# entrpn/learning-jax-sharding

Hardware: AMD Instinct MI355X
Metric: step-time ms + TFLOPS/GPU, case6 sharded attention block at 1/2/4/8 MI355X (higher is better)
Workload: dtype bf16; 1 GPU; model=case6 attention block (M=640, heads=8x64, bf16 compute, f32 params, Adam), global_batch=64, seq_len=256, parallelism=dp1, mode=train, hip_graph=True, graph_segments=1, steps_per_graph=6, warmup_steps_run=67, comm=none, grad_wire=fp32, loss=y.sum(), rules=reference

## Files before the change

learning_jax_sharding_amd/csrc/kernels/adam_common.h:

```cpp
#pragma once
#include "rowwise.h"

template <typename ST>
__device__ __forceinline__ f32x4 ld_slab4(const ST* __restrict__ p, long e) {
  if constexpr (sizeof(ST) == 4) {
    return *(const __attribute__((address_space(1))) f32x4*)(reinterpret_cast<const float*>(p) + e);
  } else {
    const u32x2 r = *(const __attribute__((address_space(1))) u32x2*)(reinterpret_cast<const bf16_t*>(p) + e);
    return unpack_bf16x4(r);
  }
}

struct AdamTensor {
  long p, g, m, v, st, sn, R, C, g_bf16, tiles_c, vec;
  long qn, sn8, qt, st8;
  long gS, g_ld, g_ss;
  long trows;
};
constexpr int kAdamMax = 32;

inline bool adam_grad_from_row(const long* r, AdamTensor& t) {
  t.g = r[1]; t.R = r[6]; t.C = r[7]; t.g_bf16 = r[8];
  t.gS = r[9]; t.g_ld = r[14]; t.g_ss = r[15];
  if (t.gS == 0) t.g_ld = t.C;
  if (t.gS > 0 && (t.g_ld < t.C || t.g_ss < 1)) return false;
  t.tiles_c = (t.C + 63) / 64;
  return true;
}
inline bool adam_grad_vec_ok(const AdamTensor& t) {
  auto al = [](long ptr, long a) { return ptr % a == 0; };
  return t.C % 4 == 0 &&
         (t.gS < 0 || (al(t.g, t.g_bf16 ? 8 : 16) && t.g_ld % 4 == 0 && (t.gS == 0 || t.g_ss % 4 == 0)));
}

template <typename ST>
__device__ __forceinline__ float slab_sum1(const ST* __restrict__ g, long gS, long ss, long i) {
  auto ld = [&](long j) {
    if constexpr (sizeof(ST) == 4) return reinterpret_cast<const float*>(g)[j];
    else return bf2f(reinterpret_cast<const bf16_t*>(g)[j]);
  };
  float acc = ld(i);
  long s = 1;
  for (; s + 3 < gS; s += 4) acc += (ld(s * ss + i) + ld((s + 1) * ss + i)) + (ld((s + 2) * ss + i) + ld((s + 3) * ss + i));
  for (; s < gS; ++s) acc += ld(s * ss + i);
  return acc;
}
template <typename ST>
__device__ __forceinline__ f32x4 slab_sum4(const ST* __restrict__ g, long gS, long ss, long i) {
  f32x4 acc = ld_slab4(g, i);
  long s = 1;
  for (; s + 3 < gS; s += 4) {
    const f32x4 v0 = ld_slab4(g, s * ss + i), v1 = ld_slab4(g, (s + 1) * ss + i);
    const f32x4 v2 = ld_slab4(g, (s + 2) * ss + i), v3 = ld_slab4(g, (s + 3) * ss + i);
    acc += (v0 + v1) + (v2 + v3);
  }
  for (; s < gS; ++s) acc += ld_slab4(g, s * ss + i);
  return acc;
}

struct StepHyper {
  float grad_scale, lr, norm, pad;
};
```

learning_jax_sharding_amd/csrc/kernels/attention.hip:

```cpp
#include "common.h"

#include <cstdlib>
#include <type_traits>

namespace {

constexpr int D = 64;
constexpr int BLK = 64;
constexpr float LOG2E = 1.4426950408889634f;
constexpr int FKR = 256;

struct FastDiv {
  unsigned m;
  int s, d;
};
static inline FastDiv make_fastdiv(int d) {
  int s = 0;
  while ((1L << s) < d) ++s;
  const unsigned long long m = ((1ULL << 32) * ((1ULL << s) - (unsigned long long)d)) / (unsigned long long)d + 1;
  return FastDiv{(unsigned)m, s, d};
}
struct AttnArgs {
  const bf16_t* q; const bf16_t* k; const bf16_t* v; const bf16_t* o; const bf16_t* dout;
  bf16_t* out;
// ... 1444 lines not shown

template <bool MASK>
__device__ __forceinline__ void fused_tile(const AttnArgs& a, const bf16_t* Qt, const bf16_t* Ot,
                                           const float* lse_s, const float* dl_s, bf16_t* dSt,
                                           const bf16x8 (&kr)[2][2], const bf16x8 (&vr)[2][2], f32x4 (&dk)[2][4],
                                           f32x4 (&dv)[2][4], int q0, int key0, int lane, const int (&offtr)[4]) {
  const int g = lane >> 4;
#pragma unroll
  for (int s2 = 0; s2 < 2; ++s2) {
    u32x4 pbu[2], sbu[2];
#pragma unroll
    for (int tt = 0; tt < 2; ++tt) {
      const int t = 2 * s2 + tt;
      const f32x4 lse = *reinterpret_cast<const f32x4*>(lse_s + 16 * t + 4 * g);
      const f32x4 ndl = *reinterpret_cast<const f32x4*>(dl_s + 16 * t + 4 * g);
      const bf16x8 q0f = frag_rows(Qt, 16 * t, 0, lane), q1f = frag_rows(Qt, 16 * t, 1, lane);
      const bf16x8 o0f = frag_rows(Ot, 16 * t, 0, lane), o1f = frag_rows(Ot, 16 * t, 1, lane);
#pragma unroll
      for (int j = 0; j < 2; ++j) {
        f32x4 s = f32x4{0.f, 0.f, 0.f, 0.f}, dp = ndl;
        s = mfma16x16x32(q0f, kr[j][0], s);
        s = mfma16x16x32(q1f, kr[j][1], s);
        dp = mfma16x16x32(o0f, vr[j][0], dp);
        dp = mfma16x16x32(o1f, vr[j][1], dp);
        float pv[4], dsv[4];
        const f32x2 sc2 = {a.scale_log2, a.scale_log2};
#pragma unroll
        for (int h = 0; h < 2; ++h) {
          const f32x2 x = pk_fms(f32x2{s[2 * h], s[2 * h + 1]}, sc2, f32x2{lse[2 * h], lse[2 * h + 1]});
          pv[2 * h] = fast_exp2(x[0]);
          pv[2 * h + 1] = fast_exp2(x[1]);
        }
        if constexpr (MASK) {
#pragma unroll
          for (int r = 0; r < 4; ++r) {
            int q = q0 + 16 * t + 4 * g + r, key = key0 + 16 * j + (lane & 15);
            bool ok = q < a.Sq && key < a.Sk && !(a.causal && key > q + a.q_offset);
            pv[r] = ok ? pv[r] : 0.f;
          }
        }
#pragma unroll
        for (int h = 0; h < 2; ++h) {
          const f32x2 d = pk_mul(f32x2{pv[2 * h], pv[2 * h + 1]}, f32x2{dp[2 * h], dp[2 * h + 1]});
          dsv[2 * h] = d[0];
          dsv[2 * h + 1] = d[1];
        }
        pbu[j][2 * tt] = pack_bf16x2(pv[0], pv[1]);
        pbu[j][2 * tt + 1] = pack_bf16x2(pv[2], pv[3]);
        sbu[j][2 * tt] = pack_bf16x2(dsv[0], dsv[1]);
        sbu[j][2 * tt + 1] = pack_bf16x2(dsv[2], dsv[3]);
        *reinterpret_cast<u32x2*>(dSt + imgS(key0 + 16 * j + (lane & 15), 4 * t + g)) =
            u32x2{sbu[j][2 * tt], sbu[j][2 * tt + 1]};
      }
    }
    bf16x8 pb[2], sb[2];
#pragma unroll
    for (int j = 0; j < 2; ++j) {
      pb[j] = __builtin_bit_cast(bf16x8, pbu[j]);
      sb[j] = __builtin_bit_cast(bf16x8, sbu[j]);
    }
#pragma unroll
    for (int dt = 0; dt < 4; ++dt) {
      bf16x8 oa = frag_tr_o(Ot, 32 * s2, offtr[dt]);
      bf16x8 qa = frag_tr_o(Qt, 32 * s2, offtr[dt]);
#pragma unroll
      for (int j = 0; j < 2; ++j) {
        dv[j][dt] = mfma16x16x32(oa, pb[j], dv[j][dt]);
        dk[j][dt] = mfma16x16x32(qa, sb[j], dk[j][dt]);
      }
    }
  }
}


__device__ __forceinline__ void fused_stamp(const AttnArgs& a, int b, int h, int wave, int lane, int k) {
#if LJS_ATTN_BWD_TRACE
  const unsigned long long t = __builtin_amdgcn_s_memtime();
  if (a.trace && lane == 0) a.trace[(((long)b * a.H + h) * (FT / 64) + wave) * 8 + k] = t;
#else
  (void)a; (void)b; (void)h; (void)wave; (void)lane; (void)k;
#endif
}

__device__ __forceinline__ void fused_delta(const bf16_t* Ot, const bf16_t* dOt, float* ndl, int tid) {
  const int row = tid >> 3, c16 = tid & 7;
  const u32x4 o = *reinterpret_cast<const u32x4*>(Ot + img16(row, c16));
  const u32x4 d = *reinterpret_cast<const u32x4*>(dOt + img16(row, c16));
  float s = dot_bf16x8(o, d);
  s += __shfl_xor(s, 1, 64);
  s += __shfl_xor(s, 2, 64);
  s += __shfl_xor(s, 4, 64);
  if (c16 == 0) ndl[row] = -s;
}

template <bool GUARD>
__device__ __forceinline__ void fused_dq(const bf16_t* Ks, const bf16_t* dSt, f32x4 (&dq)[2], int off_q,
                                         const int (&off_k)[2], int nk32) {
#pragma unroll
  for (int s2 = 0; s2 < FK / 32; ++s2) {
    if (!GUARD || s2 < nk32) {
      bf16x8 sb = frag_tr_o(dSt, 32 * s2, off_q);
#pragma unroll
      for (int i = 0; i < 2; ++i) {
        bf16x8 ka = frag_tr_o(Ks, 32 * s2, off_k[i]);
        dq[i] = mfma16x16x32(ka, sb, dq[i]);
      }
    }
  }
}

__device__ __forceinline__ void fused_dq_stage(bf16_t* img, const f32x4 (&dq)[2], float scale, int qt, int dt0,
                                               int lane) {
  const int r = 16 * qt + (lane & 15), g = lane >> 4;
#pragma unroll
  for (int i = 0; i < 2; ++i) {
    u32x2 w;
    w[0] = pack_bf16x2(dq[i][0] * scale, dq[i][1] * scale);
    w[1] = pack_bf16x2(dq[i][2] * scale, dq[i][3] * scale);
    const int c = (2 * (dt0 + i) + (g >> 1)) ^ (r & 7);
    *reinterpret_cast<u32x2*>(img + r * D + c * 8 + 4 * (g & 1)) = w;
  }
}
template <bool GUARD>
__device__ __forceinline__ void fused_dq_flush(const AttnArgs& a, const bf16_t* img, int b, int h, int q0, int tid) {
  const int r = tid >> 3, c = tid & 7;
  const u32x4 v = *reinterpret_cast<const u32x4*>(img + r * D + ((c ^ (r & 7)) << 3));
  if (!GUARD || q0 + r < a.Sq)
    *reinterpret_cast<u32x4*>(a.out3 + b * a.out3_sb + (long)(q0 + r) * a.out3_ss + h * a.out3_sh + c * 8) = v;
}

__device__ __forceinline__ void fused_dkv_out(const AttnArgs& a, bf16_t* Ks, bf16_t* Vs, const f32x4 (&dk)[2][4],
                                              const f32x4 (&dv)[2][4], int b, int h, int key0, int klim, int lane) {
#pragma unroll
  for (int j = 0; j < 2; ++j) {
    stage_rows16(Ks + key0 * D, 16 * j, dk[j], a.scale, lane);
    stage_rows16(Vs + key0 * D, 16 * j, dv[j], 1.f, lane);
  }
  flush_rows<32>(Ks + key0 * D, a.out + b * a.out_sb + h * a.out_sh, a.out_ss, key0, klim, lane);
  flush_rows<32>(Vs + key0 * D, a.out2 + b * a.out2_sb + h * a.out2_sh, a.out2_ss, key0, klim, lane);
}

template <bool KVDMA, int SW = 0>
__global__ __launch_bounds__(FT) void attn_bwd_fused_kernel(AttnArgs a) {
  __shared__ __attribute__((aligned(16))) bf16_t Ks[FK * D];
  __shared__ __attribute__((aligned(16))) bf16_t Vs[FK * D];
  __shared__ __attribute__((aligned(16))) bf16_t dSt[FK * BLK];
  __shared__ __attribute__((aligned(16))) bf16_t QO[4 * BLK * D];
  __shared__ __attribute__((aligned(16))) bf16_t Os[BLK * D];
  __shared__ __attribute__((aligned(16))) float rowc[2][2][BLK];
  __shared__ __attribute__((aligned(16))) bf16_t dQs[BLK * D];
  const int tid = threadIdx.x, lane = tid & 63, wave = tid >> 6, g = lane >> 4;
  const int h = blockIdx.x, b = blockIdx.y;
  const int key0 = wave * 32;
  auto bstamp = [&](int k) { fused_stamp(a, b, h, wave, lane, k); };
  bstamp(0);
  const bool active = key0 < a.Sk;
  const int nk32 = (a.Sk + 31) / 32;

  const bf16_t* kb = a.k + b * a.k_sb + h * a.k_sh;
  const bf16_t* vb = a.v + b * a.v_sb + h * a.v_sh;
  if constexpr (KVDMA) {
    const u32x4 rk = rsrc_u4(kb, 2 * ((long)(a.Sk - 1) * a.k_ss + D));
    const u32x4 rv = rsrc_u4(vb, 2 * ((long)(a.Sk - 1) * a.v_ss + D));
    constexpr int NWF = FT / 64;
#pragma unroll
    for (int i = 0; i < FK / 8 / NWF; ++i) {
      const int pc = wave + NWF * i;
      const int row = 8 * pc + (lane >> 3);
      const int c = ((lane & 7) ^ (((row >> 1) & 3) << 1)) * 8;
      const bool ok = row < a.Sk;
      dma_lds_x4(rk, ok ? (int)(((long)row * a.k_ss + c) * 2) : 0x7ffffff0, Ks + pc * 512);
      dma_lds_x4(rv, ok ? (int)(((long)row * a.v_ss + c) * 2) : 0x7ffffff0, Vs + pc * 512);
    }
  } else {
#pragma unroll
// ... 47 lines not shown
      vr[j][ks] = frag_rows(Vs, key0 + 16 * j, ks, lane);
    }
  const int qt = wave & 3, dt0 = 2 * (wave >> 2);
  int offtr[4];
#pragma unroll
  for (int dt = 0; dt < 4; ++dt) offtr[dt] = tr_off(16 * dt, lane);
  const int off_q = trS_off(16 * qt, lane);
  const int off_k[2] = {tr_off(16 * dt0, lane), tr_off(16 * (dt0 + 1), lane)};
  const bool wave_mask = (a.Sq % BLK) != 0 || key0 + 32 > a.Sk || a.causal;
  auto sweep = [&](auto wm, auto vs) {
    constexpr bool WM = decltype(wm)::value;
    constexpr bool VS = decltype(vs)::value;
    for (int it = 0; it < nqt; ++it) {
      const int cur = it & 1;
      const int q0 = it * BLK;
      const bool more = it + 1 < nqt;
      if (more) issue(q0 + BLK, cur ^ 1);
      const bf16_t* Qt = QO + cur * BLK * D;
      const bf16_t* Ot = QO + (2 + cur) * BLK * D;
      if (active) {
        if constexpr (WM) {
          const bool need_mask = q0 + BLK > a.Sq || key0 + 32 > a.Sk || (a.causal && key0 + 31 > q0 + a.q_offset);
          if (need_mask) fused_tile<true>(a, Qt, Ot, rowc[cur][0], rowc[cur][1], dSt, kr, vr, dk, dv, q0, key0, lane, offtr);
          else fused_tile<false>(a, Qt, Ot, rowc[cur][0], rowc[cur][1], dSt, kr, vr, dk, dv, q0, key0, lane, offtr);
        } else {
          fused_tile<false>(a, Qt, Ot, rowc[cur][0], rowc[cur][1], dSt, kr, vr, dk, dv, q0, key0, lane, offtr);
        }
      }
      asm volatile("s_waitcnt vmcnt(0)" ::: "memory");
      __syncthreads();
      if (more) finish(cur ^ 1);
      f32x4 dq[2] = {};
      if (LJS_ATTN_DQ_UNGUARD && nk32 == FK / 32) fused_dq<false>(Ks, dSt, dq, off_q, off_k, nk32);
      else fused_dq<true>(Ks, dSt, dq, off_q, off_k, nk32);
      const int qrow = q0 + 16 * qt + (lane & 15);
      if constexpr (VS) {
        fused_dq_stage(dQs, dq, a.scale, qt, dt0, lane);
      } else if (qrow < a.Sq) {
        bf16_t* rowp = a.out3 + b * a.out3_sb + (long)qrow * a.out3_ss + h * a.out3_sh;
  #pragma unroll
        for (int i = 0; i < 2; ++i) {
          u32x2 w;
          w[0] = pack_bf16x2(dq[i][0] * a.scale, dq[i][1] * a.scale);
          w[1] = pack_bf16x2(dq[i][2] * a.scale, dq[i][3] * a.scale);
          *reinterpret_cast<u32x2*>(rowp + 16 * (dt0 + i) + 4 * g) = w;
        }
      }
      __syncthreads();
      if constexpr (VS) fused_dq_flush<true>(a, dQs, b, h, q0, tid);
      if (it < 5) bstamp(2 + it);
    }
  };
  if constexpr (SW == 1) {
    (void)wave_mask;
    sweep(std::false_type{}, std::true_type{});
  } else if (a.vst == 1) {
    if (wave_mask) sweep(std::true_type{}, std::true_type{});
    else sweep(std::false_type{}, std::true_type{});
  } else {
    if (wave_mask) sweep(std::true_type{}, std::false_type{});
    else sweep(std::false_type{}, std::false_type{});
  }
  if (a.vst) {
    if (active) fused_dkv_out(a, Ks, Vs, dk, dv, b, h, key0, a.Sk, lane);
    bstamp(7);
    return;
  }
#pragma unroll
  for (int j = 0; j < 2; ++j) {
    int key = key0 + 16 * j + (lane & 15);
    if (key < a.Sk) {
      store_row_T(a.out + b * a.out_sb + (long)key * a.out_ss + h * a.out_sh, dk[j], a.scale, lane);
      store_row_T(a.out2 + b * a.out2_sb + (long)key * a.out2_ss + h * a.out2_sh, dv[j], 1.f, lane);
    }
  }
}

struct BwdProjArgs {
  const bf16_t* dy;
  const bf16_t* w;
  long dy_ld;
  int M;
  unsigned long long* steps;
};
constexpr int PJ_TS = 32;
constexpr int PJ_BK = 32;
constexpr int PJ_A = FK * PJ_BK, PJ_STAGE = PJ_A + D * PJ_BK;
constexpr int PJ_NPW = 21;
constexpr int PJ_KS = 0, PJ_VS = PJ_KS + FK * D, PJ_DST = PJ_VS + FK * D, PJ_DO = PJ_DST + FK * BLK;
constexpr int PJ_Q = PJ_DO + FK * D, PJ_OS = PJ_Q + 2 * BLK * D, PJ_ROWC = PJ_OS + BLK * D;
constexpr int PJ_LDS = PJ_ROWC + 2 * 2 * BLK * 2;
static_assert(3 * PJ_STAGE <= PJ_Q - PJ_DST, "the ring fits the dS^T and dO images");
static_assert(PJ_LDS * 2 <= 160 * 1024, "LDS");
constexpr int PJB_STAGE = D * PJ_BK;
constexpr int PJB_G = 4, PJB_AHEAD = 3, PJB_NST = (PJB_AHEAD + 1) * PJB_G;
constexpr int PJB_ROW = 2048;
static_assert((PJB_NST & (PJB_NST - 1)) == 0 && PJB_NST * PJB_STAGE <= PJ_Q - PJ_DST, "the stages fit the two images");
static_assert((PJ_LDS + PJB_ROW) * 2 <= 160 * 1024, "LDS");
template <bool BCAST>
__global__ __launch_bounds__(FT) void attn_bwd_proj_kernel(AttnArgs a, BwdProjArgs pj) {
  __shared__ __attribute__((aligned(16))) bf16_t smem[PJ_LDS + (BCAST ? PJB_ROW : 0)];
  bf16_t* const Ks = smem + PJ_KS;
  bf16_t* const Vs = smem + PJ_VS;
  bf16_t* const dSt = smem + PJ_DST;
  bf16_t* const dOi = smem + PJ_DO;
  bf16_t* const Qs = smem + PJ_Q;
  bf16_t* const Os = smem + PJ_OS;
  float* const rowc = reinterpret_cast<float*>(smem + PJ_ROWC);
  const unsigned sb = (unsigned)(uintptr_t)(LDS_PTR(const void))smem;
  const int tid = threadIdx.x, lane = tid & 63, g = lane >> 4;
  const int wave = __builtin_amdgcn_readfirstlane(tid >> 6);
  const int t = xcd_remap(blockIdx.x, gridDim.x);
  const int b = t / a.H, h = t - b * a.H;
  const int key0 = wave * 32;
  auto bstamp = [&](int k) { fused_stamp(a, b, h, wave, lane, k); };
  bstamp(0);

  const bf16_t* kb = a.k + b * a.k_sb + h * a.k_sh;
  const bf16_t* vb = a.v + b * a.v_sb + h * a.v_sh;
  const bf16_t* qb = a.q + b * a.q_sb + h * a.q_sh;
  const bf16_t* ob = a.o + b * a.o_sb + h * a.o_sh;
  const float* lse = a.lse + ((long)b * a.H + h) * FK;
  const u32x4 rk = rsrc_u4(kb, 2 * ((long)(FK - 1) * a.k_ss + D));
  const u32x4 rv = rsrc_u4(vb, 2 * ((long)(FK - 1) * a.v_ss + D));
  const u32x4 rq = rsrc_u4(qb, 2 * ((long)(FK - 1) * a.q_ss + D));
  const u32x4 ro = rsrc_u4(ob, 2 * ((long)(FK - 1) * a.o_ss + D));
  const u32x4 rl = rsrc_u4(lse, 4L * FK);
  constexpr int OOB = 0x7ffffff0;
  const int drow = 8 * wave + (lane >> 3);
  const int dchunk = ((lane & 7) ^ (((drow >> 1) & 3) << 1)) * 8;
  auto issue = [&](int q0, int buf) {
    const int r = q0 + drow;
    dma_lds_x4_at(rq, (int)(((long)r * a.q_ss + dchunk) * 2), sb + 2 * (PJ_Q + buf * BLK * D + wave * 512));
    dma_lds_x4_at(ro, (int)(((long)r * a.o_ss + dchunk) * 2), sb + 2 * (PJ_OS + wave * 512));
    if (wave == 0) dma_lds_x1_at(rl, (q0 + lane) * 4, sb + 2 * PJ_ROWC + 4 * (buf * 2 * BLK));
  };
  auto finish = [&](int buf, int blk) { fused_delta(Os, dOi + blk * BLK * D, rowc + (buf * 2 + 1) * BLK, tid); };

  {
    const int nk = pj.M / PJ_BK;
    const u32x4 ra = rsrc_u4(pj.dy + (long)b * FK * pj.dy_ld, 2 * ((long)(FK - 1) * pj.dy_ld + pj.M));
    const u32x4 rw = rsrc_u4(pj.w + (long)h * D * pj.M, 2L * D * pj.M);
    auto sstamp = [&](int k) {
#if LJS_ATTN_BWD_TRACE
      const unsigned long long ts = __builtin_amdgcn_s_memtime();
      if (pj.steps && lane == 0 && k < PJ_TS) pj.steps[(((long)b * a.H + h) * (FT / 64) + wave) * PJ_TS + k] = ts;
#else
      (void)k;
#endif
    };
    auto frag = [&](const bf16_t* img, int rb0) {
      const int row = rb0 + (lane & 15);
      return __builtin_bit_cast(bf16x8, *reinterpret_cast<const u32x4*>(
                                            img + row * PJ_BK + ((g ^ (((row >> 3) & 1) << 1)) << 3)));
    };
    f32x4 acc[BCAST ? 1 : 2][BCAST ? 1 : 4];
#pragma unroll
    for (int i = 0; i < (BCAST ? 1 : 2); ++i)
#pragma unroll
      for (int j = 0; j < (BCAST ? 1 : 4); ++j) acc[i][j] = f32x4{0.f, 0.f, 0.f, 0.f};
    const bool tw = wave < 4;
    const int pw = wave & 3;
    int va[BCAST ? 1 : 4], vw;
    if constexpr (BCAST) {
      va[0] = (pw * 512 + lane * 8) * 2;
    } else {
#pragma unroll
      for (int i = 0; i < 4; ++i) {
        const int row = 16 * (pw + 4 * i) + (lane >> 2);
        const int c = (lane & 3) ^ (((row >> 3) & 1) << 1);
        va[i] = (int)(((long)row * pj.dy_ld + 8 * c) * 2);
      }
    }
    {
      const int row = 16 * pw + (lane >> 2);
      const int c = (lane & 3) ^ (((row >> 3) & 1) << 1);
      vw = (row * pj.M + 8 * c) * 2;
    }
    const int prow = lane >> 3;
    const int pchunk = ((lane & 7) ^ (((prow >> 1) & 3) << 1)) * 8;
    auto issue_piece = [&](int j) {
      if (j < 16) {
        const int p = pw + 4 * (j >> 1);
        const int r = 8 * p + prow;
        if (j & 1) dma_lds_x4_at(rv, (int)(((long)r * a.v_ss + pchunk) * 2), sb + 2 * (PJ_VS + p * 512));
        else dma_lds_x4_at(rk, (int)(((long)r * a.k_ss + pchunk) * 2), sb + 2 * (PJ_KS + p * 512));
      } else if (j < 18) {
        const int p = pw + 4 * (j - 16);
        dma_lds_x4_at(rq, (int)(((long)(8 * p + prow) * a.q_ss + pchunk) * 2), sb + 2 * (PJ_Q + p * 512));
      } else if (j < 20) {
        const int p = pw + 4 * (j - 18);
        dma_lds_x4_at(ro, (int)(((long)(8 * p + prow) * a.o_ss + pchunk) * 2), sb + 2 * (PJ_OS + p * 512));
      } else if (pw == 0) {
        dma_lds_x1_at(rl, lane * 4, sb + 2 * PJ_ROWC);
      }
    };
    int pi = 0;
    if constexpr (BCAST) {
      const bf16_t* const rowi = smem + PJ_LDS;
      auto issue_w = [&](int kt) {
        dma_lds_x4_at(rw, kt < nk ? vw + kt * PJ_BK * 2 : OOB,
                      sb + 2 * (PJ_DST + (kt & (PJB_NST - 1)) * PJB_STAGE + pw * 512));
      };
      if (tw) {
        dma_lds_x4_at(ra, va[0], sb + 2 * (PJ_LDS + pw * 512));
#pragma unroll
        for (int kt = 0; kt < PJB_AHEAD * PJB_G; ++kt) issue_w(kt);
        static_assert(PJB_AHEAD * PJB_G == 12, "the counted wait below");
        asm volatile("s_waitcnt vmcnt(12)" ::: "memory");
      } else {
        for (; pi < PJ_NPW; ++pi) issue_piece(pi);
      }
      __builtin_amdgcn_s_barrier();
      if (tw) {
        for (int k0 = 0, gi = 0; k0 < nk; k0 += PJB_G, ++gi) {
          static_assert((PJB_AHEAD - 1) * PJB_G == 8, "the counted wait below");
          asm volatile("s_waitcnt vmcnt(8)" ::: "memory");
          asm volatile("s_waitcnt lgkmcnt(0)" ::: "memory");
          sstamp(gi);
#pragma unroll
// ... 31 lines not shown
        dma_lds_x4_at(rw, ok ? vw + ko : OOB, sb + 2 * (st + PJ_A + pw * 512));
      };
      int s0 = 0, s1 = PJ_STAGE, s2 = 2 * PJ_STAGE;
      if (tw) {
        issue_t(0, s0);
        issue_t(1, s1);
      } else {
        issue_piece(pi++);
        issue_piece(pi++);
      }
      for (int kt = 0; kt < nk; ++kt) {
        if (tw) asm volatile("s_waitcnt vmcnt(5)" ::: "memory");
        asm volatile("s_waitcnt lgkmcnt(0)" ::: "memory");
        __builtin_amdgcn_s_barrier();
        sstamp(kt);
        bf16x8 af[2], wf[4];
#pragma unroll
        for (int j = 0; j < 4; ++j) wf[j] = frag(dSt + s0 + PJ_A, 16 * j);
#pragma unroll
        for (int i = 0; i < 2; ++i) af[i] = frag(dSt + s0, 32 * wave + 16 * i);
        if (tw) issue_t(kt + 2, s2);
        else if (pi < PJ_NPW) issue_piece(pi++);
#pragma unroll
        for (int i = 0; i < 2; ++i)
#pragma unroll
          for (int j = 0; j < 4; ++j) acc[i][j] = mfma16x16x32(wf[j], af[i], acc[i][j]);
        const int sn = s0;
        s0 = s1;
        s1 = s2;
        s2 = sn;
      }
      if (!tw)
        for (; pi < PJ_NPW; ++pi) issue_piece(pi);
      asm volatile("s_waitcnt vmcnt(0)" ::: "memory");
      asm volatile("s_waitcnt lgkmcnt(0)" ::: "memory");
      __builtin_amdgcn_s_barrier();
      sstamp(nk);
#pragma unroll
      for (int i = 0; i < 2; ++i) {
        const int row = 32 * wave + 16 * i + (lane & 15);
#pragma unroll
        for (int j = 0; j < 4; ++j) {
          u32x2 w2;
          w2[0] = pack_bf16x2(acc[i][j][0], acc[i][j][1]);
          w2[1] = pack_bf16x2(acc[i][j][2], acc[i][j][3]);
          *reinterpret_cast<u32x2*>(dOi + img8(row, 4 * j + g)) = w2;
        }
      }
    }
    bstamp(6);
  }
  __syncthreads();
  finish(0, 0);
  __syncthreads();
  bstamp(1);

  f32x4 dk[2][4] = {}, dv[2][4] = {};
  bf16x8 kr[2][2], vr[2][2];
#pragma unroll
  for (int j = 0; j < 2; ++j)
#pragma unroll
    for (int ks = 0; ks < 2; ++ks) {
      kr[j][ks] = frag_rows(Ks, key0 + 16 * j, ks, lane);
      vr[j][ks] = frag_rows(Vs, key0 + 16 * j, ks, lane);
    }
  const int qt = wave & 3, dt0 = 2 * (wave >> 2);
  int offtr[4];
#pragma unroll
  for (int dt = 0; dt < 4; ++dt) offtr[dt] = tr_off(16 * dt, lane);
  const int off_q = trS_off(16 * qt, lane);
  const int off_k[2] = {tr_off(16 * dt0, lane), tr_off(16 * (dt0 + 1), lane)};
  constexpr int nqt = FK / BLK;
  for (int it = 0; it < nqt; ++it) {
    const int cur = it & 1;
    const int q0 = it * BLK;
    const bool more = it + 1 < nqt;
    if (more) issue(q0 + BLK, cur ^ 1);
    bf16_t* const dOt = dOi + it * BLK * D;
    fused_tile<false>(a, Qs + cur * BLK * D, dOt, rowc + cur * 2 * BLK, rowc + (cur * 2 + 1) * BLK, dSt, kr, vr, dk,
                      dv, q0, key0, lane, offtr);
    asm volatile("s_waitcnt vmcnt(0)" ::: "memory");
    __syncthreads();
    if (more) finish(cur ^ 1, it + 1);
    f32x4 dq[2] = {};
    fused_dq<false>(Ks, dSt, dq, off_q, off_k, FK / 32);
    fused_dq_stage(dOt, dq, a.scale, qt, dt0, lane);
    __syncthreads();
    fused_dq_flush<false>(a, dOt, b, h, q0, tid);
    bstamp(2 + it);
  }
  fused_dkv_out(a, Ks, Vs, dk, dv, b, h, key0, FK, lane);
  bstamp(7);
}

}

#define LJS_ATTN_SWITCHES(X)                                                                                  \
          \
  X(bwd_pair, 1)                                                                                              \
                                                     \
  X(dkv32, 1)                                                                                                 \
                             \
  X(dq32, 1)                                                                                                  \
                                                                             \
  X(vst, 1)                                                                                                   \
                                    \
  X(cus, 0)                                                                                                   \
                      \
  X(fwd_res, 8)                                                                                               \
                                                  \
  X(bwd_kv_dma, 2)                                                                                            \
                                                                                            \
  X(bwd_fused, 2)                                                                                             \
                                                      \
  X(bwd_proj, 2)
#define X(name, def) kSw_##name,
enum AttnSwitch { LJS_ATTN_SWITCHES(X) kSwCount };
#undef X
#define X(name, def) def,
static const int kSwDefault[kSwCount] = {LJS_ATTN_SWITCHES(X)};
static int g_sw[kSwCount] = {LJS_ATTN_SWITCHES(X)};
#undef X
LJS_API int ljs_attn_set(int which, int v) {
  if (which < 0 || which >= kSwCount) return (int)hipErrorInvalidValue;
  g_sw[which] = v < 0 ? kSwDefault[which] : v;
  return 0;
}
LJS_API int ljs_attn_get(int which) { return which < 0 || which >= kSwCount ? -1 : g_sw[which]; }
static unsigned long long* g_attn_trace = nullptr;
LJS_API void ljs_attn_set_trace(void* p) { g_attn_trace = (unsigned long long*)p; }
static unsigned long long* g_attn_trace_steps = nullptr;
LJS_API void ljs_attn_set_trace_steps(void* p) { g_attn_trace_steps = (unsigned long long*)p; }

static AttnArgs attn_args(const void* q, const void* k, const void* v, const void* o, const void* lse, const long* qs,
                          const long* ks, const long* vs, const long* os, int Sq, int Sk, int H, float scale,
                          int causal, int q_offset) {
  AttnArgs a = {};
  a.q = (const bf16_t*)q; a.k = (const bf16_t*)k; a.v = (const bf16_t*)v; a.o = (const bf16_t*)o;
  a.lse = (float*)lse;
  a.q_sb = qs[0]; a.q_ss = qs[1]; a.q_sh = qs[2];
  a.k_sb = ks[0]; a.k_ss = ks[1]; a.k_sh = ks[2];
  a.v_sb = vs[0]; a.v_ss = vs[1]; a.v_sh = vs[2];
  a.o_sb = os[0]; a.o_ss = os[1]; a.o_sh = os[2];
  a.Sq = Sq; a.Sk = Sk; a.H = H;
  a.scale = scale; a.scale_log2 = scale * LOG2E;
  a.causal = causal; a.q_offset = q_offset;
  return a;
}
static AttnArgs attn_outs(AttnArgs a, void* o1, const long* s1, void* o2 = nullptr, const long* s2 = nullptr,
                          void* o3 = nullptr, const long* s3 = nullptr) {
  a.out = (bf16_t*)o1; a.out_sb = s1[0]; a.out_ss = s1[1]; a.out_sh = s1[2];
  if (o2) { a.out2 = (bf16_t*)o2; a.out2_sb = s2[0]; a.out2_ss = s2[1]; a.out2_sh = s2[2]; }
  if (o3) { a.out3 = (bf16_t*)o3; a.out3_sb = s3[0]; a.out3_ss = s3[1]; a.out3_sh = s3[2]; }
  return a;
}
static bool none_null(std::initializer_list<const void*> ps) {
  for (const void* p : ps)
    if (!p) return false;
  return true;
}
static bool vst_ok(const void* p, long sb, long ss, long sh) {
  return (((uintptr_t)p) & 15) == 0 && sb % 8 == 0 && ss % 8 == 0 && sh % 8 == 0;
}

#define LJS_ATTN_INSTANCES(X)                    \
  X(kFwdRes8, "attn_fwd_res<8>", 512)            \
  X(kFwdRes4, "attn_fwd_res<4>", 256)            \
  X(kFwdTiled, "attn_fwd_tiled<1>", 256)         \
  X(kBwdFused00, "attn_bwd_fused<dma=0,sw=0>", FT) \
  X(kBwdFused01, "attn_bwd_fused<dma=0,sw=1>", FT) \
  X(kBwdFused10, "attn_bwd_fused<dma=1,sw=0>", FT) \
// ... 182 lines not shown
  attn_launch(p.l[0], stream, a, nullptr, p.acc_mode);
  return (int)hipGetLastError();
}

LJS_API int ljs_attn_fwd(const void* q, const void* k, const void* v, void* o, void* lse, int B, int Sq, int Sk,
                         int H, const long* qs, const long* ks, const long* vs, const long* os, float scale,
                         int causal, int q_offset, hipStream_t stream) {
  return attn_fwd_impl(q, k, v, o, lse, B, Sq, Sk, H, qs, ks, vs, os, scale, causal, q_offset, nullptr, nullptr, 0,
                       false, stream);
}

LJS_API int ljs_attn_fwd_acc(const void* q, const void* k, const void* v, void* o, void* lse, int B, int Sq, int Sk,
                             int H, const long* qs, const long* ks, const long* vs, const long* os, float scale,
                             int causal, int q_offset, void* oacc, const long* oas, int acc_mode, hipStream_t stream) {
  return attn_fwd_impl(q, k, v, o, lse, B, Sq, Sk, H, qs, ks, vs, os, scale, causal, q_offset, oacc, oas, acc_mode,
                       true, stream);
}


static int qkv_attn_fwd_impl(const void* x, long ldx, const void* w, void* qkv, void* o, void* lse, int T, int K, int N,
                             int H, float scale, void* trace, int cus, hipStream_t stream, AttnPlan* plan = nullptr) {
  QkvAttnArgs a;
  a.x = (const bf16_t*)x; a.w = (const bf16_t*)w; a.qkv = (bf16_t*)qkv; a.o = (bf16_t*)o; a.lse = (float*)lse;
  a.T = T; a.K = K; a.N = N; a.H = H; a.ldx = (int)ldx;
  a.scale_log2 = scale * LOG2E;
  a.trace = (unsigned long long*)trace;
  const AttnPlan p = qkv_attn_fwd_plan(a, ldx, cus);
  if (plan) *plan = p;
  if (plan || p.err != hipSuccess) return (int)p.err;
  ljs_launch_rec(kAttnInst[kQkvFwd].name, dim3(p.l[0].gx), p.l[0].block);
  hipLaunchKernelGGL(qkv_attn_fwd_kernel, dim3(p.l[0].gx), dim3(p.l[0].block), 0, stream, a);
  return (int)hipGetLastError();
}
LJS_API int ljs_qkv_attn_fwd(const void* x, long ldx, const void* w, void* qkv, void* o, void* lse, int T, int K, int N,
                             int H, float scale, void* trace, hipStream_t stream) {
  return qkv_attn_fwd_impl(x, ldx, w, qkv, o, lse, T, K, N, H, scale, trace, ljs_device_cus(), stream);
}

static int attn_bwd_impl(const void* q, const void* k, const void* v, const void* o, const void* dout,
                         const void* lse, void* delta, void* dq, void* dk, void* dv, int B, int Sq, int Sk, int H,
                         const long* qs, const long* ks, const long* vs, const long* os, const long* dos,
                         const long* dqs, const long* dks, const long* dvs, float scale, int causal, int q_offset,
                         hipStream_t stream, AttnPlan* plan = nullptr) {
  if (!none_null({qs, ks, vs, os, dos, dqs, dks, dvs})) return (int)hipErrorInvalidValue;
  AttnArgs a = attn_args(q, k, v, o, lse, qs, ks, vs, os, Sq, Sk, H, scale, causal, q_offset);
  a.dout = (const bf16_t*)dout;
  a.delta = (const float*)delta;
  a.do_sb = dos[0]; a.do_ss = dos[1]; a.do_sh = dos[2];
  AttnArgs f = attn_outs(a, dk, dks, dv, dvs, dq, dqs);
  const AttnPlan p = attn_bwd_plan(f, B);
  if (plan) *plan = p;
  if (plan || p.err != hipSuccess) return (int)p.err;
  if (p.l[0].inst >= kBwdFused00 && p.l[0].inst <= kBwdFused11) {
    f.vst = p.vst[0];
    f.trace = g_attn_trace;
    attn_launch(p.l[0], stream, f);
    return (int)hipGetLastError();
  }
  AttnArgs c = attn_outs(a, dq, dqs), b = attn_outs(a, dk, dks, dv, dvs);
  c.vst = p.vst[0];
  c.flags32 = p.flags32;
  b.vst = p.vst[1];
  if (p.n == 1) {
    attn_launch(p.l[0], stream, c, &b);
  } else {
    attn_launch(p.l[0], stream, c);
    attn_launch(p.l[1], stream, b);
  }
  return (int)hipGetLastError();
}
LJS_API int ljs_attn_bwd(const void* q, const void* k, const void* v, const void* o, const void* dout,
                         const void* lse, void* delta, void* dq, void* dk, void* dv, int B, int Sq, int Sk, int H,
                         const long* qs, const long* ks, const long* vs, const long* os, const long* dos,
                         const long* dqs, const long* dks, const long* dvs, float scale, int causal, int q_offset,
                         hipStream_t stream) {
  return attn_bwd_impl(q, k, v, o, dout, lse, delta, dq, dk, dv, B, Sq, Sk, H, qs, ks, vs, os, dos, dqs, dks, dvs,
                       scale, causal, q_offset, stream);
}

static int attn_bwd_proj_impl(const void* q, const void* k, const void* v, const void* o, const void* dy, long dy_ld,
                              const void* w, int M, const void* lse, void* dq, void* dk, void* dv, int B, int Sq,
                              int Sk, int H, const long* qs, const long* ks, const long* vs, const long* os,
                              const long* dqs, const long* dks, const long* dvs, float scale, int causal,
                              hipStream_t stream, AttnPlan* plan = nullptr) {
  if (!none_null({qs, ks, vs, os, dqs, dks, dvs})) return (int)hipErrorInvalidValue;
  AttnArgs a = attn_outs(attn_args(q, k, v, o, lse, qs, ks, vs, os, Sq, Sk, H, scale, causal, 0), dk, dks, dv, dvs,
                         dq, dqs);
  BwdProjArgs pj;
  pj.dy = (const bf16_t*)dy; pj.w = (const bf16_t*)w; pj.dy_ld = dy_ld; pj.M = M;
  pj.steps = g_attn_trace_steps;
  const AttnPlan p = attn_bwd_proj_plan(a, B, pj);
  if (plan) *plan = p;
  if (plan || p.err != hipSuccess) return (int)p.err;
  a.vst = p.vst[0];
  a.trace = g_attn_trace;
  ljs_launch_rec(kAttnInst[kBwdProj].name, dim3(p.l[0].gx), p.l[0].block);
  const bool bcast = dy_ld == 0 && M <= PJB_ROW && bwd_proj_bcast_on();
  g_bwd_proj_last_path = bcast;
  if (bcast) hipLaunchKernelGGL(attn_bwd_proj_kernel<true>, dim3(p.l[0].gx), dim3(p.l[0].block), 0, stream, a, pj);
  else hipLaunchKernelGGL(attn_bwd_proj_kernel<false>, dim3(p.l[0].gx), dim3(p.l[0].block), 0, stream, a, pj);
  return (int)hipGetLastError();
}
LJS_API int ljs_attn_bwd_proj_last_path() { return g_bwd_proj_last_path; }
LJS_API int ljs_attn_bwd_proj(const void* q, const void* k, const void* v, const void* o, const void* dy, long dy_ld,
                              const void* w, int M, const void* lse, void* dq, void* dk, void* dv, int B, int Sq,
                              int Sk, int H, const long* qs, const long* ks, const long* vs, const long* os,
                              const long* dqs, const long* dks, const long* dvs, float scale, int causal,
                              hipStream_t stream) {
  return attn_bwd_proj_impl(q, k, v, o, dy, dy_ld, w, M, lse, dq, dk, dv, B, Sq, Sk, H, qs, ks, vs, os, dqs, dks, dvs,
                            scale, causal, stream);
}

LJS_API int ljs_attn_plan(int kind, int B, int Sq, int Sk, int H, int causal, int acc_mode, void* const* addr,
                          const long* st, int M, long ld, int K, int cus, int* out, char* names, int cap) {
  void* const* p = addr;
  AttnPlan pl = attn_reject();
  if (kind == 0 || kind == 1)
    attn_fwd_impl(p[0], p[1], p[2], p[3], p[4], B, Sq, Sk, H, st, st + 3, st + 6, st + 9, 1.f, causal, 0, p[7],
                  kind ? st + 15 : nullptr, acc_mode, kind == 1, nullptr, &pl);
  else if (kind == 2)
    attn_bwd_impl(p[0], p[1], p[2], p[3], p[5], p[4], p[6], p[8], p[9], p[10], B, Sq, Sk, H, st, st + 3, st + 6, st + 9,
                  st + 12, st + 18, st + 21, st + 24, 1.f, causal, 0, nullptr, &pl);
  else if (kind == 3)
    attn_bwd_proj_impl(p[0], p[1], p[2], p[3], p[11], ld, p[12], M, p[4], p[8], p[9], p[10], B, Sq, Sk, H, st, st + 3,
                       st + 6, st + 9, st + 18, st + 21, st + 24, 1.f, causal, nullptr, &pl);
  else if (kind == 4)
    qkv_attn_fwd_impl(p[0], ld, p[1], p[2], p[3], p[4], B * Sq, K, M, H, 1.f, nullptr, cus, nullptr, &pl);
  const int v[16] = {(int)pl.err, pl.n, pl.l[0].inst, (int)pl.l[0].gx, (int)pl.l[0].gy, (int)pl.l[0].block,
                     pl.l[1].inst, (int)pl.l[1].gx, (int)pl.l[1].gy, (int)pl.l[1].block, pl.vst[0], pl.vst[1],
                     pl.flags32, pl.nw, pl.nqb, pl.acc_mode};
  for (int i = 0; i < 16; ++i) out[i] = v[i];
  if (names && cap > 0)
    snprintf(names, (size_t)cap, "%s%s%s", pl.n > 0 ? kAttnInst[pl.l[0].inst].name : "", pl.n > 1 ? " " : "",
             pl.n > 1 ? kAttnInst[pl.l[1].inst].name : "");
  return (int)pl.err;
}
```

learning_jax_sharding_amd/csrc/kernels/clip.hip:

```cpp
#include "adam_common.h"
#include <algorithm>
#include <math.h>

namespace {

constexpr int kSumsqRows = 32, kSumsqThreads = 256, kSumsqMaxBlocks = 1024, kSumsqSlots = 64;
constexpr int kSumsqTicketWord = kSumsqMaxBlocks;
constexpr int kSumsqSlotWord = kSumsqTicketWord + 64;
constexpr int kSumsqWsWords = kSumsqSlotWord + 2 * kSumsqSlots;
static_assert(1 + kSumsqMaxBlocks / (int)kTicketGroup <= 64 && kSumsqSlotWord % 2 == 0, "workspace layout");

struct SumsqBatch {
  AdamTensor t[kAdamMax];
  int tile_start[kAdamMax + 1];
  int n;
};

__device__ __forceinline__ void add_sq4(float& acc, const f32x4& g) {
#pragma unroll
  for (int e = 0; e < 4; ++e) acc += g[e] * g[e];
}

__global__ __launch_bounds__(kSumsqThreads) void grad_sumsq_kernel(SumsqBatch batch, float* __restrict__ partials,
                                                                    unsigned* __restrict__ tickets,
                                                                    double* __restrict__ slot) {
  const int lane = threadIdx.x & 63, w = threadIdx.x >> 6;
  const int c4 = (threadIdx.x & 15) * 4, r0 = threadIdx.x >> 4;
  const int total = batch.tile_start[batch.n];
  float acc = 0.f;
  for (int id = blockIdx.x; id < total; id += gridDim.x) {
    int ti = 0;
#pragma unroll
    for (int i = 1; i < kAdamMax; ++i) ti += (i < batch.n && id >= batch.tile_start[i]) ? 1 : 0;
    const AdamTensor& T = batch.t[ti];
    const long R = T.R, C = T.C, gS = T.gS, g_ld = T.g_ld, g_ss = T.g_ss;
    const bool bf = T.g_bf16 != 0;
    const int local = id - batch.tile_start[ti];
    const int tr_i = local / (int)T.tiles_c, tc_i = local % (int)T.tiles_c;
    if (gS >= 0 && T.vec && (long)(tc_i + 1) * 64 <= C) {
      const long cbase = (long)tc_i * 64 + c4;
      f32x4 g[2];
      bool ok[2];
#pragma unroll
      for (int q = 0; q < 2; ++q) {
        const long row = (long)tr_i * kSumsqRows + r0 + 16 * q;
        ok[q] = row < R;
        const long gi = (ok[q] ? row : 0) * g_ld + cbase;
        if (gS > 0) {
          g[q] = bf ? slab_sum4(reinterpret_cast<const bf16_t*>(T.g), gS, g_ss, gi)
                    : slab_sum4(reinterpret_cast<const float*>(T.g), gS, g_ss, gi);
        } else {
          g[q] = bf ? ld_slab4(reinterpret_cast<const bf16_t*>(T.g), gi)
                    : ld_slab4(reinterpret_cast<const float*>(T.g), gi);
        }
      }
#pragma unroll
      for (int q = 0; q < 2; ++q)
        if (ok[q]) add_sq4(acc, g[q]);
      continue;
    }
    const long col = (long)tc_i * 64 + lane;
#pragma unroll 4
    for (int rr = 0; rr < kSumsqRows / 4; ++rr) {
      const long row = (long)tr_i * kSumsqRows + w + 4 * rr;
      if (row < R && col < C) {
        const long gi = row * g_ld + col;
        const float g = gS > 0   ? (bf ? slab_sum1(reinterpret_cast<const bf16_t*>(T.g), gS, g_ss, gi)
                                       : slab_sum1(reinterpret_cast<const float*>(T.g), gS, g_ss, gi))
                        : gS < 0 ? __int_as_float((int)g_ld)
                        : bf     ? bf2f(reinterpret_cast<const bf16_t*>(T.g)[gi])
                                 : reinterpret_cast<const float*>(T.g)[gi];
        acc += g * g;
      }
    }
  }
  acc = warp_sum64(acc);
  __shared__ float part[kSumsqThreads / 64];
  if (lane == 0) part[w] = acc;
  __syncthreads();
  if (w != 0) return;
  if (lane == 0) {
    float t = part[0];
#pragma unroll
    for (int k = 1; k < kSumsqThreads / 64; ++k) t += part[k];
    sc1_store(partials + blockIdx.x, t);
  }
  if (!wave_last_2lvl(tickets, blockIdx.x, gridDim.x)) return;
  constexpr int kRounds = kSumsqMaxBlocks / 64;
  __shared__ float parked[kSumsqMaxBlocks];
  float v[kRounds];
#pragma unroll
  for (int r = 0; r < kRounds; ++r) {
    const unsigned i = r * 64 + lane;
    v[r] = i < gridDim.x ? sc1_load(partials + i) : 0.f;
  }
#pragma unroll
  for (int r = 0; r < kRounds; ++r) parked[r * 64 + lane] = v[r];
  double sum = 0.0;
#pragma unroll 1
  for (unsigned r = 0; r * 64 < gridDim.x; ++r) {
    const unsigned x = __float_as_uint(parked[r * 64 + lane]);
#pragma unroll
    for (int l = 0; l < 64; ++l) sum += (double)__uint_as_float(__builtin_amdgcn_readlane(x, l));
  }
  if (lane == 0) *slot = sum;
}

struct SchedArgs {
  int kind;
  double p[5];
};
__device__ __forceinline__ double sched_linear(double init, double end, double steps, double begin, double count) {
  if (steps <= 0.0) return init;
  const double c = fmin(fmax(count - begin, 0.0), steps);
  return (init - end) * (1.0 - c / steps) + end;
}
__device__ __forceinline__ double sched_cosine(double init, double decay_steps, double alpha, double count) {
  const double c = fmin(count, decay_steps);
  return init * ((1.0 - alpha) * 0.5 * (1.0 + cos(M_PI * c / decay_steps)) + alpha);
}
__device__ __forceinline__ double sched_value(const SchedArgs& s, double count) {
  switch (s.kind) {
    case 1: return sched_linear(s.p[0], s.p[1], s.p[2], s.p[3], count);
    case 2: return sched_cosine(s.p[0], s.p[1], s.p[2], count);
    case 3: return count < s.p[2] ? sched_linear(s.p[0], s.p[1], s.p[2], 0.0, count)
                                  : sched_cosine(s.p[1], s.p[3], s.p[4], count - s.p[2]);
    default: return s.p[0];
  }
}

__global__ __launch_bounds__(64) void step_hyper_kernel(const double* __restrict__ slots, int n_slots,
                                                        const double* __restrict__ gathered, int n_gathered,
                                                        double* __restrict__ partial_out, const int* __restrict__ step,
                                                        int step_offset, int clip, double max_norm, SchedArgs sched,
                                                        StepHyper* __restrict__ rec) {
  double s = 0.0;
  for (int i = 0; i < n_slots; ++i) s += slots[i];
  if (partial_out) {
    if (threadIdx.x == 0) *partial_out = s;
    return;
  }
  if (gathered) {
    s = 0.0;
    for (int i = 0; i < n_gathered; ++i) s += gathered[i];
  }
  const double norm = sqrt(s);
  const double scale = (!clip || norm < max_norm) ? 1.0 : max_norm / norm;
  const double count = (double)(*step + step_offset - 1);
  const double lr = sched_value(sched, count);
  if (threadIdx.x == 0) {
    rec->grad_scale = (float)scale;
// ... 51 lines not shown
```

learning_jax_sharding_amd/csrc/kernels/elementwise.hip:

```cpp
#include "adam_common.h"
#include <stdlib.h>
#include <type_traits>
#include <algorithm>

namespace {

constexpr int kMaxGrid = 2048;

inline int grid_for(long n, int per_block) {
  long g = (n + per_block - 1) / per_block;
  if (g < 1) g = 1;
  return (int)(g > kMaxGrid ? kMaxGrid : g);
}

__global__ void cast_f32_bf16(const float* __restrict__ in, bf16_t* __restrict__ out, long n) {
  long i8 = ((long)blockIdx.x * blockDim.x + threadIdx.x) * 8;
  long stride = (long)gridDim.x * blockDim.x * 8;
  for (; i8 + 8 <= n; i8 += stride) {
    float v[8];
    load_chunk8(in + i8, v);
    store_chunk(out + i8, v);
  }
  if (i8 < n) for (long j = i8; j < n; ++j) out[j] = f2bf(in[j]);
}
// ... 367 lines not shown
  int lane = threadIdx.x & 63;
  if (row >= rows) return;
  const float* x = in + row * L;
  float* y = out + row * L;
  float m = -INFINITY;
  for (int i = lane; i < L; i += 64) m = fmaxf(m, x[i]);
  m = warp_max64(m);
  float s = 0.f;
  for (int i = lane; i < L; i += 64) s += __expf(x[i] - m);
  s = warp_sum64(s);
  float inv = 1.f / s;
  for (int i = lane; i < L; i += 64) y[i] = __expf(x[i] - m) * inv;
}

template <typename G>
__global__ void adam_kernel(const float* __restrict__ p, const G* __restrict__ g, const float* __restrict__ m,
                            const float* __restrict__ v, float* __restrict__ po, float* __restrict__ mo,
                            float* __restrict__ vo, const int* __restrict__ step, long n, float lr, float b1,
                            float b2, float eps, float wd) {
  const float t = (float)(*step);
  const float bc1 = 1.f - powf(b1, t), bc2 = 1.f - powf(b2, t);
  const float inv_bc1 = 1.f / bc1, inv_sqrt_bc2 = rsqrtf(bc2);
  long i = ((long)blockIdx.x * blockDim.x + threadIdx.x) * 4;
  long stride = (long)gridDim.x * blockDim.x * 4;
  for (; i < n; i += stride) {
    if (i + 4 <= n) {
      f32x4 pp = *reinterpret_cast<const f32x4*>(p + i);
      f32x4 mm = *reinterpret_cast<const f32x4*>(m + i);
      f32x4 vv = *reinterpret_cast<const f32x4*>(v + i);
      f32x4 gg;
#pragma unroll
      for (int k = 0; k < 4; ++k) gg[k] = load1(g + i + k);
#pragma unroll
      for (int k = 0; k < 4; ++k) {
        mm[k] = b1 * mm[k] + (1.f - b1) * gg[k];
        vv[k] = b2 * vv[k] + (1.f - b2) * gg[k] * gg[k];
        float u = (mm[k] * inv_bc1) / (sqrtf(vv[k]) * inv_sqrt_bc2 + eps) + wd * pp[k];
        pp[k] -= lr * u;
      }
      *reinterpret_cast<f32x4*>(po + i) = pp;
      *reinterpret_cast<f32x4*>(mo + i) = mm;
      *reinterpret_cast<f32x4*>(vo + i) = vv;
    } else {
      for (long j = i; j < n; ++j) {
        float gg = load1(g + j);
        float mm = b1 * m[j] + (1.f - b1) * gg;
        float vv = b2 * v[j] + (1.f - b2) * gg * gg;
        float u = (mm * inv_bc1) / (sqrtf(vv) * inv_sqrt_bc2 + eps) + wd * p[j];
        po[j] = p[j] - lr * u;
        mo[j] = mm;
        vo[j] = vv;
      }
    }
  }
}

#ifndef LJS_ADAM_SLAB_DB
#define LJS_ADAM_SLAB_DB 1
#endif
struct AdamBatch {
  AdamTensor t[kAdamMax];
  int tile_start[kAdamMax + 1];
  int n;
};


struct CastJob {
  const float* src;
  bf16_t* dst;
  long n;
};

__device__ __forceinline__ float scaled_grad(float g, float scale) {
  g *= scale;
  asm volatile("" : "+v"(g));
  return g;
}

template <int kAdamRows, int kThreads, bool kDyn = false>
__global__ __launch_bounds__(kThreads) void adam_multi_kernel(AdamBatch batch, int* __restrict__ step, int step_offset,
                                                         std::conditional_t<kDyn, const StepHyper*, float> lr_arg,
                                                         float b1, float b2, float eps, float wd, CastJob cast) {
  __shared__ float tr[kAdamRows][65];
  float lr;
  [[maybe_unused]] float gscale = 1.f;
  if constexpr (kDyn) {
    gscale = lr_arg->grad_scale;
    lr = lr_arg->lr;
  } else {
    lr = lr_arg;
  }
  const int id = blockIdx.x;
  if (cast.n > 0 && id >= batch.tile_start[batch.n]) {
    const int cb = id - batch.tile_start[batch.n], ncb = (int)gridDim.x - batch.tile_start[batch.n];
    long i8 = ((long)cb * kThreads + threadIdx.x) * 8;
    const long stride = (long)ncb * kThreads * 8;
    for (; i8 + 8 <= cast.n; i8 += stride) {
      float v[8];
      load_chunk8(cast.src + i8, v);
      store_chunk(cast.dst + i8, v);
    }
    if (i8 < cast.n)
      for (long j = i8; j < cast.n; ++j) cast.dst[j] = f2bf(cast.src[j]);
    return;
  }
  int ti = 0;
#pragma unroll
  for (int i = 1; i < kAdamMax; ++i) ti += (i < batch.n && id >= batch.tile_start[i]) ? 1 : 0;
  const AdamTensor T = batch.t[ti];
  const int local = id - batch.tile_start[ti];
  const int tr_i = local / (int)T.tiles_c, tc_i = local % (int)T.tiles_c;
  const int s0 = *step;
  const float t = (float)(s0 + step_offset);
  const float inv_bc1 = 1.f / (1.f - powf(b1, t)), inv_sqrt_bc2 = rsqrtf(1.f - powf(b2, t));
  float* P = reinterpret_cast<float*>(T.p);
  float* Mm = reinterpret_cast<float*>(T.m);
  float* Vv = reinterpret_cast<float*>(T.v);
  const int tx = threadIdx.x & 63, ty = threadIdx.x >> 6;
  const int col = tc_i * 64 + tx;
  constexpr int RPP = kThreads / 16;
  auto vec_tile = [&](auto nq_tag) {
    constexpr int NQ = decltype(nq_tag)::value;
    constexpr int TR = RPP * NQ;
    static_assert(NQ >= 1 && TR <= kAdamRows, "tile height");
    const int c4 = (threadIdx.x & 15) * 4, r0 = threadIdx.x >> 4;
    const long cbase = (long)tc_i * 64 + c4;
    f32x4 gv[NQ], mv[NQ], vv[NQ], pv[NQ];
    bool ok[NQ];
    long gix[NQ];
#pragma unroll
    for (int q = 0; q < NQ; ++q) {
      const int row = tr_i * TR + r0 + RPP * q;
      ok[q] = row < T.R;
      gix[q] = ok[q] ? (long)row * T.g_ld + cbase : cbase;
      const long i = ok[q] ? (long)row * T.C + cbase : cbase;
      mv[q] = *(const __attribute__((address_space(1))) f32x4*)(Mm + i);
      vv[q] = *(const __attribute__((address_space(1))) f32x4*)(Vv + i);
      pv[q] = *(const __attribute__((address_space(1))) f32x4*)(P + i);
    }
    if (T.gS > 0) {
      auto slab_sum = [&](auto tag) {
        using ST = decltype(tag);
        const ST* G = reinterpret_cast<const ST*>(T.g);
#pragma unroll
        for (int q = 0; q < NQ; ++q) gv[q] = ld_slab4(G, gix[q]);
        long s = 1;
#if LJS_ADAM_SLAB_DB
        const long full = NQ <= 2 ? 1 + ((T.gS - 1) / 4) * 4 : 1;
        if (s < full) {
          f32x4 va[NQ][4], vb[NQ][4];
          auto load = [&](f32x4 (&v)[NQ][4], long s0) {
#pragma unroll
            for (int q = 0; q < NQ; ++q)
#pragma unroll
              for (int j = 0; j < 4; ++j) v[q][j] = ld_slab4(G, (s0 + j) * T.g_ss + gix[q]);
          };
          auto add = [&](f32x4 (&v)[NQ][4]) {
#pragma unroll
            for (int q = 0; q < NQ; ++q) gv[q] += (v[q][0] + v[q][1]) + (v[q][2] + v[q][3]);
          };
          load(va, s);
          for (;;) {
            if (s + 4 < full) load(vb, s + 4);
            add(va);
            s += 4;
            if (s >= full) break;
            if (s + 4 < full) load(va, s + 4);
            add(vb);
            s += 4;
            if (s >= full) break;
          }
        }
#endif
        for (; s + 3 < T.gS; s += 4) {
          f32x4 v[NQ][4];
#pragma unroll
          for (int q = 0; q < NQ; ++q)
#pragma unroll
            for (int j = 0; j < 4; ++j) v[q][j] = ld_slab4(G, (s + j) * T.g_ss + gix[q]);
#pragma unroll
          for (int q = 0; q < NQ; ++q) gv[q] += (v[q][0] + v[q][1]) + (v[q][2] + v[q][3]);
        }
        if (NQ <= 2 && s < T.gS) {
          f32x4 r[NQ][3];
#pragma unroll
          for (int j = 0; j < 3; ++j)
            if (s + j < T.gS) {
#pragma unroll
              for (int q = 0; q < NQ; ++q) r[q][j] = ld_slab4(G, (s + j) * T.g_ss + gix[q]);
            }
#pragma unroll
          for (int j = 0; j < 3; ++j)
            if (s + j < T.gS) {
#pragma unroll
              for (int q = 0; q < NQ; ++q) gv[q] += r[q][j];
            }
          s = T.gS;
        }
        for (; s < T.gS; ++s) {
#pragma unroll
          for (int q = 0; q < NQ; ++q) gv[q] += ld_slab4(G, s * T.g_ss + gix[q]);
        }
      };
      if (T.g_bf16) slab_sum(bf16_t{});
      else slab_sum(float{});
    }
#pragma unroll
    for (int q = 0; q < NQ; ++q) {
      const long gi = gix[q];
      if (T.gS > 0) {
      } else if (T.gS < 0) {
        const float c = __int_as_float((int)T.g_ld);
        gv[q] = f32x4{c, c, c, c};
      } else if (T.g_bf16) {
        const u32x2 raw = *reinterpret_cast<const u32x2*>(reinterpret_cast<const bf16_t*>(T.g) + gi);
        gv[q] = unpack_bf16x4(raw);
      } else {
        gv[q] = *reinterpret_cast<const f32x4*>(reinterpret_cast<const float*>(T.g) + gi);
      }
    }
#pragma unroll
    for (int q = 0; q < NQ; ++q) {
      const int rl = r0 + RPP * q;
#pragma unroll
      for (int e = 0; e < 4; ++e) {
        float g = gv[q][e];
        if constexpr (kDyn) g = scaled_grad(g, gscale);
        const float m = b1 * mv[q][e] + (1.f - b1) * g;
        const float v = b2 * vv[q][e] + (1.f - b2) * g * g;
        const float p = pv[q][e];
        mv[q][e] = m;
        vv[q][e] = v;
        pv[q][e] = p - lr * ((m * inv_bc1) / (sqrtf(v) * inv_sqrt_bc2 + eps) + wd * p);
        tr[rl][c4 + e] = pv[q][e];
      }
      if (ok[q]) {
        const long i = (long)(tr_i * TR + rl) * T.C + cbase;
        *reinterpret_cast<f32x4*>(P + i) = pv[q];
        *reinterpret_cast<f32x4*>(Mm + i) = mv[q];
        *reinterpret_cast<f32x4*>(Vv + i) = vv[q];
        if (T.sn)
          *reinterpret_cast<u32x2*>(reinterpret_cast<bf16_t*>(T.sn) + i) =
              u32x2{pack_bf16x2(pv[q][0], pv[q][1]), pack_bf16x2(pv[q][2], pv[q][3])};
      }
      if (T.qn) {
        float amax = fmaxf(fmaxf(fabsf(pv[q][0]), fabsf(pv[q][1])), fmaxf(fabsf(pv[q][2]), fabsf(pv[q][3])));
        amax = fmaxf(amax, __shfl_xor(amax, 1, 64));
        amax = fmaxf(amax, __shfl_xor(amax, 2, 64));
        amax = fmaxf(amax, __shfl_xor(amax, 4, 64));
        const int x = mx_exponent(amax);
        const float inv = ldexpf(1.f, -x);
        if (ok[q]) {
          const long i = (long)(tr_i * TR + rl) * T.C + cbase;
          *reinterpret_cast<unsigned*>(reinterpret_cast<unsigned char*>(T.qn) + i) =
              pack4_e4m3(pv[q][0] * inv, pv[q][1] * inv, pv[q][2] * inv, pv[q][3] * inv);
          if ((threadIdx.x & 7) == 0) reinterpret_cast<unsigned char*>(T.sn8)[i / 32] = (unsigned char)(x + 127);
        }
      }
    }
    if (T.st || T.qt) {
      __syncthreads();
      constexpr int RL = TR / 4;
      const int r4 = (threadIdx.x % RL) * 4, cl0 = threadIdx.x / RL;
      const int orow0 = tc_i * 64, ocol = tr_i * TR + r4;
      const bool rows_vec = (T.R & 3) == 0 && ocol + 4 <= T.R;
      static_assert(kThreads / RL <= 64, "transpose pass wider than the tile");
#pragma unroll
      for (int q = 0; q < 64 / (kThreads / RL); ++q) {
        const int cl = cl0 + (kThreads / RL) * q, c = orow0 + cl;
        if (T.st) {
          bf16_t* dst = reinterpret_cast<bf16_t*>(T.st) + (long)c * T.R + ocol;
          if (rows_vec) {
            *reinterpret_cast<u32x2*>(dst) = u32x2{pack_bf16x2(tr[r4][cl], tr[r4 + 1][cl]),
                                                   pack_bf16x2(tr[r4 + 2][cl], tr[r4 + 3][cl])};
          } else {
            for (int k = 0; k < 4 && ocol + k < T.R; ++k) dst[k] = f2bf(tr[r4 + k][cl]);
          }
        }
        if (T.qt) {
          const float a0 = tr[r4][cl], a1 = tr[r4 + 1][cl], a2 = tr[r4 + 2][cl], a3 = tr[r4 + 3][cl];
          float amax = fmaxf(fmaxf(fabsf(a0), fabsf(a1)), fmaxf(fabsf(a2), fabsf(a3)));
          amax = fmaxf(amax, __shfl_xor(amax, 1, 64));
          amax = fmaxf(amax, __shfl_xor(amax, 2, 64));
          amax = fmaxf(amax, __shfl_xor(amax, 4, 64));
          const int x = mx_exponent(amax);
          const float inv = ldexpf(1.f, -x);
          const long o = (long)c * T.R + ocol;
          *reinterpret_cast<unsigned*>(reinterpret_cast<unsigned char*>(T.qt) + o) =
              pack4_e4m3(a0 * inv, a1 * inv, a2 * inv, a3 * inv);
          if ((threadIdx.x & 7) == 0) reinterpret_cast<unsigned char*>(T.st8)[o / 32] = (unsigned char)(x + 127);
        }
      }
    }
  };
  if (T.vec && (tc_i + 1) * 64 <= T.C) {
    if constexpr (RPP == 16) {
      if (T.trows == 16) vec_tile(std::integral_constant<int, 1>{});
      else if (kAdamRows >= 32 && T.trows == 32) vec_tile(std::integral_constant<int, (kAdamRows >= 32 ? 2 : 1)>{});
      else vec_tile(std::integral_constant<int, kAdamRows / RPP>{});
    } else {
      vec_tile(std::integral_constant<int, kAdamRows / RPP>{});
    }
    return;
  }
#pragma unroll 4
  for (int rr = 0; rr < kAdamRows / (kThreads / 64); ++rr) {
    const int rl = ty + (kThreads / 64) * rr, row = tr_i * kAdamRows + rl;
    float newp = 0.f;
    if (row < T.R && col < T.C) {
      const long i = (long)row * T.C + col;
      const long gi = (long)row * T.g_ld + col;
      float g = T.gS > 0   ? (T.g_bf16 ? slab_sum1(reinterpret_cast<const bf16_t*>(T.g), T.gS, T.g_ss, gi)
                                        : slab_sum1(reinterpret_cast<const float*>(T.g), T.gS, T.g_ss, gi))
                : T.gS < 0 ? __int_as_float((int)T.g_ld)
                : T.g_bf16 ? bf2f(reinterpret_cast<const bf16_t*>(T.g)[gi])
                           : reinterpret_cast<const float*>(T.g)[gi];
      if constexpr (kDyn) g = scaled_grad(g, gscale);
      float m = b1 * Mm[i] + (1.f - b1) * g;
      float v = b2 * Vv[i] + (1.f - b2) * g * g;
      float p = P[i];
      newp = p - lr * ((m * inv_bc1) / (sqrtf(v) * inv_sqrt_bc2 + eps) + wd * p);
      P[i] = newp;
      Mm[i] = m;
      Vv[i] = v;
      if (T.sn) reinterpret_cast<bf16_t*>(T.sn)[i] = f2bf(newp);
    }
    tr[rl][tx] = newp;
  }
  if (T.st) {
    __syncthreads();
    const int orow0 = tc_i * 64;
    for (int idx = threadIdx.x; idx < kAdamRows * 64; idx += kThreads) {
      const int r = idx % kAdamRows, cl = idx / kAdamRows, c = orow0 + cl, ocol = tr_i * kAdamRows + r;
      if (c < T.C && ocol < T.R) reinterpret_cast<bf16_t*>(T.st)[(long)c * T.R + ocol] = f2bf(tr[r][cl]);
    }
  }
}

struct RngRegion {
  long start[8];
  long size[8];
  long gstride[8];
  int ndim;
};

__device__ __forceinline__ void philox10(unsigned& c0, unsigned& c1, unsigned& c2, unsigned& c3, unsigned k0,
                                         unsigned k1) {
#pragma unroll
  for (int r = 0; r < 10; ++r) {
    unsigned long long p0 = (unsigned long long)0xD2511F53u * c0;
    unsigned long long p1 = (unsigned long long)0xCD9E8D57u * c2;
    unsigned hi0 = (unsigned)(p0 >> 32), lo0 = (unsigned)p0;
    unsigned hi1 = (unsigned)(p1 >> 32), lo1 = (unsigned)p1;
    unsigned n0 = hi1 ^ c1 ^ k0, n2 = hi0 ^ c3 ^ k1;
    c0 = n0; c1 = lo1; c2 = n2; c3 = lo0;
    k0 += 0x9E3779B9u;
    k1 += 0xBB67AE85u;
  }
}

__device__ __forceinline__ double u01(unsigned x) { return ((double)(x >> 8) + 0.5) * (1.0 / 16777216.0); }

template <typename T>
__global__ void rng_kernel(T* __restrict__ out, RngRegion reg, long n, unsigned k0, unsigned k1, int dist, float lo,
                           float hi, float erf_a, float erf_b) {
  long i = (long)blockIdx.x * blockDim.x + threadIdx.x;
  long stride = (long)gridDim.x * blockDim.x;
  for (; i < n; i += stride) {
    long rem = i, gidx = 0;
    for (int d = reg.ndim - 1; d >= 0; --d) {
      long li = rem % reg.size[d];
      rem /= reg.size[d];
      gidx += (reg.start[d] + li) * reg.gstride[d];
    }
    unsigned c0 = (unsigned)gidx, c1 = (unsigned)(gidx >> 32), c2 = 0, c3 = 0;
    philox10(c0, c1, c2, c3, k0, k1);
    float val;
    if (dist == 0) {
      double u1 = u01(c0), u2 = u01(c1);
      val = (float)(sqrt(-2.0 * log(u1)) * cos(6.283185307179586 * u2));
    } else if (dist == 1) {
      val = (float)(lo + (hi - lo) * u01(c0));
    } else {
      double u = erf_a + (erf_b - erf_a) * u01(c0);
      double z = 1.4142135623730951 * erfinv(u);
      val = (float)fmin(fmax(z, (double)lo), (double)hi);
    }
    if constexpr (sizeof(T) == 4) out[i] = val;
    else out[i] = f2bf(val);
  }
}

template <typename T>
__global__ void dropout_kernel(const T* __restrict__ x, T* __restrict__ y, RngRegion reg, long n, unsigned k0,
                               unsigned k1, float keep) {
  long i = (long)blockIdx.x * blockDim.x + threadIdx.x;
// ... 234 lines not shown
    long per = 256L * (is_bf16 ? 8 : 4) * 16;
    int g = grid_for(n, (int)per);
    if (g > kMaxSumBlocks) g = kMaxSumBlocks;
    if (is_bf16)
      hipLaunchKernelGGL(sum_all_ticket_kernel<bf16_t>, dim3(g), dim3(256), 0, s, (const bf16_t*)in, n, partials,
                         ticket, out, out_bf16);
    else
      hipLaunchKernelGGL(sum_all_ticket_kernel<float>, dim3(g), dim3(256), 0, s, (const float*)in, n, partials,
                         ticket, out, out_bf16);
    return (int)hipGetLastError();
  }
  if (out_bf16) return (int)hipErrorInvalidValue;
  (void)hipMemsetAsync(out, 0, sizeof(float), s);
  int g = grid_for(n, 256 * 16);
  if (is_bf16)
    hipLaunchKernelGGL(sum_all_kernel<bf16_t>, dim3(g), dim3(256), 0, s, (const bf16_t*)in, n, (float*)out);
  else
    hipLaunchKernelGGL(sum_all_kernel<float>, dim3(g), dim3(256), 0, s, (const float*)in, n, (float*)out);
  return (int)hipGetLastError();
}

constexpr long kColsumWsFloats = 1L << 20;
LJS_API long ljs_colsum_ws_floats() { return kColsumWsFloats; }
LJS_API int ljs_colsum(const void* in, int is_bf16, int R, int C, long ld, void* out, int accumulate, void* ws,
                       hipStream_t s) {
  if (ld == 0) {
    hipLaunchKernelGGL(colsum_bcast_kernel, dim3((C + 255) / 256), dim3(256), 0, s, in, is_bf16, R, C, (float*)out,
                       accumulate);
    return (int)hipGetLastError();
  }
  if (is_bf16 && C % 8 == 0 && ld % 8 == 0 && (((uintptr_t)in) & 15) == 0) {
    int cb = (C + 63) / 64;
    int want = 512 / cb;
    int gy = want < 1 ? 1 : want;
    int rpb = (R + gy - 1) / gy;
    if (rpb < 32) rpb = 32;
    gy = (R + rpb - 1) / rpb;
    if (ws && cb <= 4096 && (long)gy * C + 4096 <= kColsumWsFloats) {
      hipLaunchKernelGGL(colsum_ticket_kernel, dim3(cb, gy), dim3(256), 0, s, (const bf16_t*)in, R, C, ld, rpb,
                         (float*)ws + 4096, (unsigned*)ws, (float*)out, accumulate, (const bf16_t*)nullptr, 0L,
                         (bf16_t*)nullptr);
      return (int)hipGetLastError();
    }
    if (!accumulate) (void)hipMemsetAsync(out, 0, sizeof(float) * C, s);
    hipLaunchKernelGGL(colsum_vec_kernel, dim3(cb, gy), dim3(256), 0, s, (const bf16_t*)in, R, C, ld, rpb,
                       (float*)out);
    return (int)hipGetLastError();
  }
  if (!accumulate) (void)hipMemsetAsync(out, 0, sizeof(float) * C, s);
  int gy = R / 256;
  if (gy < 1) gy = 1;
  if (gy > 64) gy = 64;
  dim3 grid((C + 255) / 256, gy);
  if (is_bf16)
    hipLaunchKernelGGL(colsum_kernel<bf16_t>, grid, dim3(256), 0, s, (const bf16_t*)in, R, C, ld, (float*)out);
  else
    hipLaunchKernelGGL(colsum_kernel<float>, grid, dim3(256), 0, s, (const float*)in, R, C, ld, (float*)out);
  return (int)hipGetLastError();
}

LJS_API int ljs_slab_reduce(const void* slabs, int S, long slab_stride, int R, int C, void* out, int cb, long out_bs,
                            int accumulate, void* out_bf16, void* tail, void* tail_bf16, int tail_n, float tail_val,
                            int slabs_bf16, hipStream_t s) {
  if (tail_n < 0 || (tail_n > 0 && !tail)) return (int)hipErrorInvalidValue;
  if (C % 4 || cb % 4 || C % cb || slab_stride % 4 || out_bs % 4 || S < 1 || (((uintptr_t)slabs) & 15) ||
      (((uintptr_t)out) & 15))
    return (int)hipErrorInvalidValue;
  const long n4 = (long)R * C / 4;
  int grid = (int)((n4 + 255) / 256);
  if (grid > 2048) grid = 2048;
  if (grid < 1) grid = 1;
  if (out_bf16 && (((uintptr_t)out_bf16) & 7)) return (int)hipErrorInvalidValue;
  if (slabs_bf16)
    hipLaunchKernelGGL(slab_reduce_kernel<bf16_t>, dim3(grid), dim3(256), 0, s, (const bf16_t*)slabs, S, slab_stride,
                       R, C, (float*)out, cb, out_bs, accumulate, (bf16_t*)out_bf16, (float*)tail,
                       (bf16_t*)tail_bf16, tail_n, tail_val);
  else
    hipLaunchKernelGGL(slab_reduce_kernel<float>, dim3(grid), dim3(256), 0, s, (const float*)slabs, S, slab_stride, R,
                       C, (float*)out, cb, out_bs, accumulate, (bf16_t*)out_bf16, (float*)tail, (bf16_t*)tail_bf16,
                       tail_n, tail_val);
  return (int)hipGetLastError();
}

LJS_API int ljs_bcast_scalar(const void* g, int g_bf16, int C, float R, void* row, void* db, void* db_bf16,
                             hipStream_t s) {
  hipLaunchKernelGGL(bcast_scalar_kernel, dim3((C + 255) / 256), dim3(256), 0, s, g, g_bf16, C, R, (bf16_t*)row,
                     (float*)db, (bf16_t*)db_bf16);
  return (int)hipGetLastError();
}

struct PadBox {
  long full[6], lo[6], size[6], sstride[6];
  int nd;
};
template <typename T>
__global__ __launch_bounds__(256) void pad_box_kernel(const T* __restrict__ src, T* __restrict__ out, PadBox b,
                                                      long total) {
  if (b.nd == 1 && total < (1L << 31)) {
    const int lo = (int)b.lo[0], n = (int)b.size[0], ss = (int)b.sstride[0];
    for (int i = blockIdx.x * 256 + threadIdx.x; i < (int)total; i += gridDim.x * 256) {
      const int rel = i - lo;
      out[i] = (rel >= 0 && rel < n) ? src[rel * ss] : T(0);
    }
    return;
  }
  for (long i = blockIdx.x * 256L + threadIdx.x; i < total; i += (long)gridDim.x * 256) {
    long r = i, so = 0;
    bool in = true;
    for (int d = b.nd - 1; d >= 0; --d) {
      const long c = r % b.full[d];
      r /= b.full[d];
      const long rel = c - b.lo[d];
      in = in && rel >= 0 && rel < b.size[d];
      so += rel * b.sstride[d];
    }
    out[i] = in ? src[so] : T(0);
  }
}

LJS_API int ljs_pad_box(const void* src, void* out, int nd, const long* full, const long* lo, const long* size,
                        const long* sstride, int esize, hipStream_t s) {
  if (nd < 1 || nd > 6) return (int)hipErrorInvalidValue;
  PadBox b;
  long total = 1;
  for (int d = 0; d < nd; ++d) {
    b.full[d] = full[d];
    b.lo[d] = lo[d];
    b.size[d] = size[d];
    b.sstride[d] = sstride[d];
    total *= full[d];
  }
  b.nd = nd;
  if (total == 0) return 0;
  long grid = (total + 255) / 256;
  if (grid > 4096) grid = 4096;
  if (esize == 2)
    hipLaunchKernelGGL(pad_box_kernel<unsigned short>, dim3(grid), dim3(256), 0, s, (const unsigned short*)src,
                       (unsigned short*)out, b, total);
  else if (esize == 4)
    hipLaunchKernelGGL(pad_box_kernel<unsigned>, dim3(grid), dim3(256), 0, s, (const unsigned*)src, (unsigned*)out, b,
                       total);
  else if (esize == 8)
    hipLaunchKernelGGL(pad_box_kernel<unsigned long long>, dim3(grid), dim3(256), 0, s,
                       (const unsigned long long*)src, (unsigned long long*)out, b, total);
  else
    return (int)hipErrorInvalidValue;
  return (int)hipGetLastError();
}

LJS_API int ljs_sum_partials(const void* p, int n, void* out, int out_bf16, hipStream_t s) {
  hipLaunchKernelGGL(sum_partials_kernel, dim3(1), dim3(256), 0, s, (const float*)p, n, out, out_bf16);
  return (int)hipGetLastError();
}

LJS_API int ljs_relu_bwd_colsum(const void* in, const void* mask, int R, int C, long ld, long mld, void* masked_out,
                                void* out, void* ws, hipStream_t s) {
  if (C % 8 || ld % 8 || mld % 8 || (((uintptr_t)in) & 15) || (((uintptr_t)mask) & 15) || (((uintptr_t)masked_out) & 15) || !ws)
    return (int)hipErrorInvalidValue;
  int cb = (C + 63) / 64;
  int want = 512 / cb;
  int gy = want < 1 ? 1 : want;
  int rpb = (R + gy - 1) / gy;
  if (rpb < 32) rpb = 32;
  gy = (R + rpb - 1) / rpb;
  if (cb > 4096 || (long)gy * C + 4096 > kColsumWsFloats) return (int)hipErrorInvalidValue;
  hipLaunchKernelGGL(colsum_ticket_kernel, dim3(cb, gy), dim3(256), 0, s, (const bf16_t*)in, R, C, ld, rpb,
// ... 263 lines not shown
```

learning_jax_sharding_amd/ops/hip.py:

```python
from __future__ import annotations

import contextlib
import ctypes
import math
import os
import threading
from typing import Dict, List, Optional, Sequence

import torch

__all__ = ["lib", "available", "gemm", "bmm_nt", "linear", "attention", "cast", "sum_all", "softmax_lastdim",
           "adam", "rng_fill", "colsum", "supports_cast", "norm", "xent", "xent_stats", "embed",
           "embed_grad", "rope", "swiglu"]

_HERE = os.path.dirname(os.path.abspath(__file__))
_LIBPATH = os.environ.get("LJS_KERNELS_LIB") or os.path.join(os.path.dirname(_HERE), "_lib", "libljs_kernels.so")
_LIB = None
_LOCK = threading.Lock()

c_void_p, c_int, c_long, c_float, c_uint = ctypes.c_void_p, ctypes.c_int, ctypes.c_long, ctypes.c_float, ctypes.c_uint
c_double = ctypes.c_double
_LP = ctypes.POINTER(ctypes.c_long)

_SIGS = {
    "ljs_pack_rows": [c_void_p, c_int, c_void_p, c_long, c_long, c_long, c_int, c_void_p, c_void_p],
    "ljs_gemm_group_end": [c_void_p],
    "ljs_gemm_bf16": [c_void_p, c_void_p, c_void_p, c_void_p, c_int, c_int, c_int, c_long, c_long, c_long, c_long,
                      c_long, c_long, c_long, c_int, c_int, c_int, c_int, c_int, c_float, c_int, c_int, c_void_p,
                      ctypes.POINTER(c_int), c_void_p, c_long, c_long, c_void_p],
    "ljs_gemm_plan": [c_void_p, c_void_p, c_void_p, c_void_p, c_int, c_int, c_int, c_long, c_long, c_long, c_long,
                      c_long, c_long, c_long, c_int, c_int, c_int, c_int, c_int, c_float, c_int, c_int, c_void_p,
                      ctypes.POINTER(c_int), c_void_p, c_long, c_long, c_int, ctypes.POINTER(c_int), ctypes.c_char_p,
                      c_int],
    "ljs_sum_partials": [c_void_p, c_int, c_void_p, c_int, c_void_p],
    "ljs_mse_colsum_ws_bytes": [c_int, c_int],
    "ljs_gemm_f32": [c_void_p, c_void_p, c_void_p, c_int, c_int, c_int, c_long, c_long, c_long, c_long, c_long,
                     c_long, c_long, c_long, c_int, c_void_p],
    "ljs_attn_fwd": [c_void_p, c_void_p, c_void_p, c_void_p, c_void_p, c_int, c_int, c_int, c_int, _LP, _LP, _LP, _LP,
                     c_float, c_int, c_int, c_void_p],
    "ljs_attn_set_trace": [c_void_p],
    "ljs_attn_set_trace_steps": [c_void_p],
    "ljs_qkv_attn_fwd": [c_void_p, c_long, c_void_p, c_void_p, c_void_p, c_void_p, c_int, c_int, c_int, c_int, c_float,
                         c_void_p, c_void_p],
    "ljs_attn_fwd_acc": [c_void_p, c_void_p, c_void_p, c_void_p, c_void_p, c_int, c_int, c_int, c_int, _LP, _LP, _LP,
                         _LP, c_float, c_int, c_int, c_void_p, _LP, c_int, c_void_p],
    "ljs_attn_bwd": [c_void_p, c_void_p, c_void_p, c_void_p, c_void_p, c_void_p, c_void_p, c_void_p, c_void_p,
                     c_void_p, c_int, c_int, c_int, c_int, _LP, _LP, _LP, _LP, _LP, _LP, _LP, _LP, c_float, c_int,
                     c_int, c_void_p],
    "ljs_attn_bwd_proj": [c_void_p, c_void_p, c_void_p, c_void_p, c_void_p, c_long, c_void_p, c_int, c_void_p,
                          c_void_p, c_void_p, c_void_p, c_int, c_int, c_int, c_int, _LP, _LP, _LP, _LP, _LP, _LP, _LP,
                          c_float, c_int, c_void_p],
    "ljs_attn_bwd_proj_enabled": [c_int, c_int],
    "ljs_attn_bwd_proj_last_path": [],
    "ljs_cast_f32_bf16": [c_void_p, c_void_p, c_long, c_void_p],
    "ljs_cast_bf16_f32": [c_void_p, c_void_p, c_long, c_void_p],
    "ljs_swap01_bf16": [c_void_p, c_int, c_void_p, c_int, c_int, c_int, c_void_p],
    "ljs_transpose_bf16": [c_void_p, c_void_p, c_int, c_int, c_long, c_long, c_void_p],
    "ljs_sum_n": [ctypes.POINTER(c_void_p), c_int, c_int, c_long, c_void_p, c_void_p],
    "ljs_rows_sum_f32": [c_void_p, c_int, c_int, c_long, c_void_p, c_void_p],
    "ljs_cast_transpose_f32_bf16": [c_void_p, c_void_p, c_int, c_int, c_long, c_long, c_void_p],
    "ljs_sum_all": [c_void_p, c_int, c_long, c_void_p, c_int, c_void_p, c_void_p],
    "ljs_colsum": [c_void_p, c_int, c_int, c_int, c_long, c_void_p, c_int, c_void_p, c_void_p],
    "ljs_fill_row_bf16": [c_void_p, c_int, c_void_p, c_long, c_void_p],
    "ljs_relu_bwd_colsum": [c_void_p, c_void_p, c_int, c_int, c_long, c_long, c_void_p, c_void_p, c_void_p, c_void_p],
    "ljs_relu_bwd": [c_void_p, c_void_p, c_int, c_int, c_long, c_long, c_void_p, c_void_p],
    "ljs_bcast_scalar": [c_void_p, c_int, c_int, c_float, c_void_p, c_void_p, c_void_p, c_void_p],
    "ljs_pad_box": [c_void_p, c_void_p, c_int, _LP, _LP, _LP, _LP,
                    c_int, c_void_p],
    "ljs_slab_reduce": [c_void_p, c_int, c_long, c_int, c_int, c_void_p, c_int, c_long, c_int, c_void_p, c_void_p,
                        c_void_p, c_int, c_float, c_int, c_void_p],
    "ljs_softmax_rows_f32": [c_void_p, c_void_p, c_long, c_int, c_void_p],
    "ljs_adam_f32": [c_void_p, c_void_p, c_int, c_void_p, c_void_p, c_void_p, c_void_p, c_void_p, c_void_p, c_long,
                     c_float, c_float, c_float, c_float, c_float, c_void_p],
    "ljs_adam_multi": [_LP, c_int, c_void_p, c_int, c_void_p, c_float, c_float, c_float, c_float, c_float,
                       c_void_p, c_void_p, c_long, c_void_p],
    "ljs_adam_multi_dyn": [_LP, c_int, c_void_p, c_int, c_void_p, c_float, c_float, c_float, c_float,
                           c_void_p, c_void_p, c_long, c_void_p],
    "ljs_grad_sumsq": [_LP, c_int, c_void_p, c_int, c_void_p],
    "ljs_grad_sumsq_ws_words": [],
    "ljs_grad_sumsq_slot_word": [],
    "ljs_grad_sumsq_slots": [],
    "ljs_step_hyper": [c_void_p, c_int, c_void_p, c_int, c_void_p, c_void_p, c_int, c_int, c_double, c_int,
                       c_double, c_double, c_double, c_double, c_double, c_void_p, c_void_p],
    "ljs_step_add": [c_void_p, c_int, c_void_p],
    "ljs_adam_set_rows": [c_int],
    "ljs_clock_probe": [c_void_p, c_void_p, c_uint, c_uint, c_void_p],
    "ljs_mse_loss": [c_void_p, c_void_p, c_int, c_long, c_float, c_void_p, c_void_p, c_void_p, c_void_p],
    "ljs_mse_colsum": [c_void_p, c_void_p, c_int, c_int, c_int, c_float, c_void_p, c_void_p, c_void_p, c_void_p,
                       c_void_p],
    "ljs_rng_fill": [c_void_p, c_int, c_int, _LP, _LP, _LP, c_uint, c_uint, c_int, c_float, c_float, c_float,
                     c_float, c_void_p],
    "ljs_dropout": [c_void_p, c_void_p, c_int, c_int, _LP, _LP, _LP, c_uint, c_uint, c_float, c_void_p],
    "ljs_norm_fwd": [c_void_p, c_int, c_long, c_void_p, c_void_p, c_void_p, c_int, c_long, c_void_p, c_void_p, c_int,
                     c_int, c_float, c_int, c_void_p],
    "ljs_norm_bwd": [c_void_p, c_int, c_long, c_void_p, c_int, c_long, c_void_p, c_void_p, c_void_p, c_void_p, c_long,
                     c_int, c_int, c_int, c_void_p, c_void_p, c_void_p, c_void_p],
    "ljs_norm_bwd_ws_bytes": [c_int, c_int],
    "ljs_xent_fwd": [c_void_p, c_int, c_long, c_void_p, c_int, c_long, c_void_p, c_void_p, c_void_p, c_void_p, c_long,
                     c_int, c_void_p],
    "ljs_xent_bwd": [c_void_p, c_int, c_long, c_void_p, c_int, c_long, c_void_p, c_void_p, c_void_p, c_void_p, c_void_p,
                     c_long, c_long, c_int, c_void_p],
    "ljs_xent_wave_max_v": [],
    "ljs_embed_fwd": [c_void_p, c_int, c_long, c_void_p, c_int, c_long, c_void_p, c_int, c_long, c_int, c_int, c_void_p],
    "ljs_embed_index": [c_void_p, c_int, c_long, c_long, c_int, c_void_p, c_void_p, c_void_p, c_void_p, c_void_p, c_int,
                        c_void_p],
    "ljs_embed_scan": [c_void_p, c_int, c_void_p, c_void_p, c_int, c_void_p],
    "ljs_embed_bwd": [c_void_p, c_int, c_long, c_int, c_int, c_void_p, c_void_p, c_void_p, c_int, c_void_p, c_void_p,
                      c_void_p],
    "ljs_embed_chunk": [],
    "ljs_embed_allpairs_max_tokens": [],
    "ljs_embed_work_cap": [c_long],
    "ljs_rope": [c_void_p, c_void_p, c_void_p, c_void_p, c_int, c_int, c_int, c_int, c_int, c_int, _LP, _LP, _LP, _LP,
                 c_void_p, c_void_p, c_long, c_long, c_int, c_void_p],
    "ljs_rope_set_max_blocks": [c_int],
    "ljs_swiglu": [c_void_p, c_void_p, c_void_p, c_int, c_int, c_int, c_int, c_int, _LP, _LP, _LP, c_void_p],
    "ljs_swiglu_bwd": [c_void_p, c_void_p, c_void_p, c_void_p, c_void_p, c_int, c_int, c_int, c_int, c_int, _LP, _LP,
                       _LP, _LP, _LP, c_void_p],
    "ljs_swiglu_set_max_blocks": [c_int],
    "ljs_launch_count": [],
    "ljs_launch_get": [c_long, ctypes.c_char_p, c_int],
    "ljs_attn_set": [c_int, c_int],
    "ljs_attn_get": [c_int],
    "ljs_attn_plan": [c_int, c_int, c_int, c_int, c_int, c_int, c_int, ctypes.POINTER(c_void_p), _LP, c_int, c_long,
                      c_int, c_int, ctypes.POINTER(c_int), ctypes.c_char_p, c_int],
}


def lib():
    global _LIB
    if _LIB is None:
        with _LOCK:
            if _LIB is None:
                if not os.path.exists(_LIBPATH):
                    raise RuntimeError(
                        f"HIP kernel library not found at {_LIBPATH}: build it with "
                        "`python -m learning_jax_sharding_amd.csrc.build` (or __graft_entry__.build())")
                L = ctypes.CDLL(_LIBPATH)
                for name, argt in _SIGS.items():
                    fn = getattr(L, name)
                    fn.argtypes = argt
                    fn.restype = c_int
                L.ljs_mse_colsum_ws_bytes.restype = c_long
                L.ljs_norm_bwd_ws_bytes.restype = c_long
                L.ljs_launch_count.restype = c_long
                for name in ("ljs_grad_sumsq_ws_words", "ljs_grad_sumsq_slot_word", "ljs_grad_sumsq_slots"):
                    getattr(L, name).restype = c_long
                _LIB = L
    return _LIB


def _launch_at(i: int) -> Optional[dict]:
    buf = ctypes.create_string_buffer(256)
    if lib().ljs_launch_get(i, buf, len(buf)) < 0:
# ... 1577 lines not shown
        return torch.empty((S, B, H, D), dtype=dtype, device=ref.device).permute(1, 0, 2, 3)
    return torch.empty(shape, dtype=dtype, device=ref.device)


_ATTN_KINDS = ("fwd", "fwd_acc", "bwd", "bwd_proj", "qkv_fwd")
_ATTN_ADDRS = ("q", "k", "v", "o", "lse", "dout", "delta", "oacc", "dq", "dk", "dv", "dy", "w")
_ATTN_STRIDES = ("q", "k", "v", "o", "dout", "oacc", "dq", "dk", "dv")


def attn_plan(kind: str, B: int, Sq: int, Sk: int, H: int, *, causal: bool = False, q_offset: int = 0,
              acc_mode: int = 0, strides=None, addrs=None, M: int = 0, dy_ld: int = 0, K: int = 0, N=None, ldx=None,
              cus: int = 256) -> dict:
    strides, addrs, order = strides or {}, addrs or {}, _ATTN_ADDRS
    if kind == "qkv_fwd":
        M, dy_ld, order = 64 * H if N is None else N, K if ldx is None else ldx, ("x", "w", "qkv", "o", "lse")
    rows = {"k": Sk, "v": Sk, "dk": Sk, "dv": Sk}
    st = [s for n in _ATTN_STRIDES for s in strides.get(n) or (rows.get(n, Sq) * H * 64, H * 64, 64)]
    ad = (c_void_p * len(order))(*[addrs.get(n, 4096) for n in order])
    out, names = (c_int * 16)(), ctypes.create_string_buffer(96)
    lib().ljs_attn_plan(_ATTN_KINDS.index(kind), B, Sq, Sk, H, int(causal), acc_mode, ad, _longs(st), M, dy_ld, K,
                        cus, out, names, len(names))
    launches = [{"name": n, "grid": (out[3 + 4 * i], out[4 + 4 * i], 1), "blocks": out[3 + 4 * i] * out[4 + 4 * i],
                 "block": out[5 + 4 * i], "acc_mode": None if out[15] < 0 else out[15]}
                for i, n in enumerate(names.value.decode().split())]
    return {"err": out[0], "launches": launches, "vst": (out[10], out[11]), "flags32": out[12], "nw": out[13],
            "nqb": out[14]}


_FUSED_ATTN: Dict[tuple, tuple] = {}


def qkv_attn_fwd(xb: torch.Tensor, wt: torch.Tensor, out: torch.Tensor, H: int, scale: float,
                 trace: Optional[torch.Tensor] = None):
    T, K = xb.shape
    N = wt.shape[1]
    assert (xb.dtype == torch.bfloat16 and wt.dtype == torch.bfloat16 and out.dtype == torch.bfloat16
            and xb.stride(1) == 1 and wt.is_contiguous() and out.is_contiguous() and out.shape == (T, 3 * N)
            and wt.shape == (3, N, K) and N == 64 * H and T % 256 == 0 and K % 128 == 0)
    o = torch.empty((T, N), dtype=torch.bfloat16, device=xb.device)
    lse = torch.empty((T // 256, H, 256), dtype=torch.float32, device=xb.device)
    _ck(lib().ljs_qkv_attn_fwd(_p(xb), xb.stride(0), _p(wt), _p(out), _p(o), _p(lse), T, K, N, H, float(scale),
                               _p(trace) if trace is not None else None, _stream(xb)), "ljs_qkv_attn_fwd")
    return o, lse


def _fused_key(t: torch.Tensor, scale: float):
    return (t.data_ptr(), t._version, t.device.index, float(scale))


def clear_fused_attention() -> None:
    _FUSED_ATTN.clear()


def register_fused_attention(out: torch.Tensor, o: torch.Tensor, lse: torch.Tensor, H: int, scale: float) -> None:
    from ..spmd import graphs as _graphs
    if clear_fused_attention not in _graphs.AFTER_CAPTURE:
        _graphs.AFTER_CAPTURE.append(clear_fused_attention)
    _FUSED_ATTN.clear()
    _FUSED_ATTN[_fused_key(out, scale)] = (o, lse, tuple(out.shape), H)


def _take_fused_attention(q, k, v, scale, causal, q_offset):
    if not _FUSED_ATTN or causal or q_offset:
        return None
    ent = _FUSED_ATTN.get(_fused_key(q, scale))
    if ent is None:
        return None
    o, lse, (T, N3), H = ent
    N = N3 // 3
    B, S = T // 256, 256
    es = q.element_size()
    if not (q.shape == (B, S, H, 64) and k.shape == q.shape and v.shape == q.shape
            and q.stride() == (S * N3, N3, 64, 1) and k.stride() == q.stride() and v.stride() == q.stride()
            and k.data_ptr() == q.data_ptr() + N * es and v.data_ptr() == q.data_ptr() + 2 * N * es):
        return None
    del _FUSED_ATTN[_fused_key(q, scale)]
    FUSED_ATTN_STATS["taken"] += 1
    return o.view(B, S, H, 64), lse


FUSED_ATTN_STATS = {"taken": 0}


_PROJ_PENDING: Dict[int, tuple] = {}
ATTN_BWD_PROJ_STATS = {"taken": 0, "materialised": 0}


def proj_shape_ok(B: int, Sq: int, Sk: int, H: int, D: int, M: int, dy_ld: int, causal: bool) -> bool:
    return D == 64 and attn_plan("bwd_proj", B, Sq, Sk, H, causal=causal, M=M, dy_ld=dy_ld)["err"] == 0


def attn_bwd_proj_ok(q, k, v, o, dy: torch.Tensor, dy_ld: int, w: torch.Tensor, causal: bool, outs=None) -> bool:
    B, Sq, H, D = q.shape
    ts = dict(zip(("q", "k", "v", "o", "dq", "dk", "dv"), (q, k, v, o) + tuple(outs or ())))
    if not (D == 64 and w.shape[0] == H * D and dy.dtype == torch.bfloat16 and w.dtype == torch.bfloat16
            and w.is_contiguous() and all(t.dtype == torch.bfloat16 and t.stride(3) == 1 for t in ts.values())):
        return False
    addrs = {n: t.data_ptr() for n, t in ts.items()}
    addrs.update(dy=dy.data_ptr(), w=w.data_ptr())
    return attn_plan("bwd_proj", B, Sq, k.shape[1], H, causal=causal, M=w.shape[1], dy_ld=dy_ld, addrs=addrs,
                     strides={n: _strides3(t) for n, t in ts.items()})["err"] == 0


def attn_bwd_proj_block(q, k, v, o, dy: torch.Tensor, dy_ld: int, w: torch.Tensor, lse, scale: float,
                        causal: bool = False, outs=None):
    B, Sq, H, D = q.shape
    if outs is None:
        outs = tuple(torch.empty((B, Sq, H, D), dtype=torch.bfloat16, device=q.device) for _ in range(3))
    dq, dk, dv = outs
    rc = lib().ljs_attn_bwd_proj(_p(q), _p(k), _p(v), _p(o), _p(dy), int(dy_ld), _p(w), int(w.shape[1]), _p(lse),
                                 _p(dq), _p(dk), _p(dv), B, Sq, k.shape[1], H, _longs(_strides3(q)),
                                 _longs(_strides3(k)), _longs(_strides3(v)), _longs(_strides3(o)),
                                 _longs(_strides3(dq)), _longs(_strides3(dk)), _longs(_strides3(dv)), float(scale),
                                 int(causal), _stream(q))
    _ck(rc, "ljs_attn_bwd_proj")
    return dq, dk, dv


def attn_bwd_proj_last_path() -> int:
    return lib().ljs_attn_bwd_proj_last_path()


def defer_out_proj(dy: torch.Tensor, ld: int, wn: torch.Tensor, dx: torch.Tensor, launch) -> None:
    from ..spmd import graphs as _graphs
    if materialise_out_proj not in _graphs.BEFORE_CUT:
        _graphs.BEFORE_CUT.append(materialise_out_proj)
        _graphs.AFTER_CAPTURE.append(materialise_out_proj)
    _PROJ_PENDING[dx.data_ptr()] = (dy, ld, wn, dx, launch)


def materialise_out_proj() -> None:
    while _PROJ_PENDING:
        _, ent = _PROJ_PENDING.popitem()
        ent[4]()
        ATTN_BWD_PROJ_STATS["materialised"] += 1


def _take_out_proj(do: torch.Tensor, q, k, v, o, outs, causal):
    ent = _PROJ_PENDING.pop(do.data_ptr(), None)
    if ent is None:
        return None
    dy, ld, wn, dx, launch = ent
    B, Sq, H, D = q.shape
    if (do.dtype == torch.bfloat16 and tuple(do.shape) == (B, Sq, H, D) and do.is_contiguous()
            and dx.numel() == do.numel() and attn_bwd_proj_ok(q, k, v, o, dy, ld, wn, causal, outs)):
        ATTN_BWD_PROJ_STATS["taken"] += 1
        return dy, ld, wn
    launch()
    ATTN_BWD_PROJ_STATS["materialised"] += 1
    return None


def _attn_fwd_call(q, k, v, o, lse, scale, causal, q_offset):
    B, Sq, H, _ = q.shape
    _ck(lib().ljs_attn_fwd(_p(q), _p(k), _p(v), _p(o), _p(lse), B, Sq, k.shape[1], H, _longs(_strides3(q)),
                           _longs(_strides3(k)), _longs(_strides3(v)), _longs(_strides3(o)), scale, int(causal),
                           q_offset, _stream(q)), "ljs_attn_fwd")
    return o, lse


def _lse_like(q: torch.Tensor) -> torch.Tensor:
    return torch.empty((q.shape[0], q.shape[2], q.shape[1]), dtype=torch.float32, device=q.device)


def _bf16_rows(do: torch.Tensor) -> torch.Tensor:
    do = do.to(torch.bfloat16)
    return do if do.stride(3) == 1 else do.contiguous()


def _attn_bwd_call(q, k, v, o, do, lse, dq, dk, dv, scale, causal, q_offset):
    B, Sq, H, _ = q.shape
    delta = torch.empty((B, H, Sq), dtype=torch.float32, device=q.device)
    _ck(lib().ljs_attn_bwd(_p(q), _p(k), _p(v), _p(o), _p(do), _p(lse), _p(delta), _p(dq), _p(dk), _p(dv), B, Sq,
                           k.shape[1], H, _longs(_strides3(q)), _longs(_strides3(k)), _longs(_strides3(v)),
                           _longs(_strides3(o)), _longs(_strides3(do)), _longs(_strides3(dq)), _longs(_strides3(dk)),
                           _longs(_strides3(dv)), scale, int(causal), q_offset, _stream(q)), "ljs_attn_bwd")


class _Attention(torch.autograd.Function):
    @staticmethod
    def forward(ctx, q, k, v, scale, causal, q_offset):
        pre = _take_fused_attention(q, k, v, scale, causal, q_offset)
        if pre is not None:
            o, lse = pre
        else:
            o, lse = _attn_fwd_call(q, k, v, _bs_like(q.shape, q), _lse_like(q), scale, causal, q_offset)
        ctx.save_for_backward(q, k, v, o, lse)
        ctx.args = (scale, causal, q_offset)
        return o

    @staticmethod
    def backward(ctx, do):
        q, k, v, o, lse = ctx.saved_tensors
        scale, causal, q_offset = ctx.args
        B, Sq, H, D = q.shape
        Sk = k.shape[1]
        do = _bf16_rows(do)
        st = q.stride()
        fused = (Sq == Sk and k.stride() == st and v.stride() == st and st[3] == 1 and st[2] == D
                 and k.data_ptr() - q.data_ptr() == H * D * 2 and v.data_ptr() - q.data_ptr() == 2 * H * D * 2
                 and st[1] == 3 * H * D and st[0] == Sq * st[1])
        if fused:
            dqkv = torch.empty((B, Sq, 3, H, D), dtype=torch.bfloat16, device=q.device)
            dq, dk, dv = dqkv[:, :, 0], dqkv[:, :, 1], dqkv[:, :, 2]
        else:
            dq = _bs_like((B, Sq, H, D), q)
            dk = _bs_like((B, Sk, H, D), k)
            dv = _bs_like((B, Sk, H, D), v)
        proj = _take_out_proj(do, q, k, v, o, (dq, dk, dv), causal) if _PROJ_PENDING else None
        if proj is not None:
            attn_bwd_proj_block(q, k, v, o, proj[0], proj[1], proj[2], lse, scale, causal, outs=(dq, dk, dv))
        else:
            _attn_bwd_call(q, k, v, o, do, lse, dq, dk, dv, scale, causal, q_offset)
        return dq.to(q.dtype), dk.to(k.dtype), dv.to(v.dtype), None, None, None


def attn_fwd_lse(q, k, v, scale: float, causal: bool = False, q_offset: int = 0):
    o = torch.empty(q.shape, dtype=torch.bfloat16, device=q.device)
    return _attn_fwd_call(q, k, v, o, _lse_like(q), scale, causal, q_offset)


def attn_fwd_acc(q, k, v, scale: float, causal: bool, q_offset: int, oacc: torch.Tensor, lse: torch.Tensor, mode: int,
                 out: Optional[torch.Tensor] = None):
    B, Sq, H, D = q.shape
    Sk = k.shape[1]
    assert oacc.dtype == torch.float32 and oacc.stride(3) == 1 and lse.dtype == torch.float32
    if mode == 3 and out is None:
        out = _bs_like((B, Sq, H, D), q)
    o = out if out is not None else q
    rc = lib().ljs_attn_fwd_acc(_p(q), _p(k), _p(v), _p(o), _p(lse), B, Sq, Sk, H, _longs(_strides3(q)),
                                _longs(_strides3(k)), _longs(_strides3(v)), _longs(_strides3(o)), scale, int(causal),
                                q_offset, _p(oacc), _longs(_strides3(oacc)), int(mode), _stream(q))
    _ck(rc, "ljs_attn_fwd_acc")
    return out


def attn_bwd_block(q, k, v, o, do, lse, scale: float, causal: bool = False, q_offset: int = 0):
    B, Sq, H, D = q.shape
    Sk = k.shape[1]
    dq = torch.empty((B, Sq, H, D), dtype=torch.bfloat16, device=q.device)
    dk = torch.empty((B, Sk, H, D), dtype=torch.bfloat16, device=q.device)
    dv = torch.empty((B, Sk, H, D), dtype=torch.bfloat16, device=q.device)
    _attn_bwd_call(q, k, v, o, _bf16_rows(do), lse, dq, dk, dv, scale, causal, q_offset)
    return dq, dk, dv


def attention(q, k, v, scale: float, causal: bool = False, q_offset: int = 0) -> torch.Tensor:
    ok = (q.shape[-1] == 64 and k.shape[-1] == 64 and v.shape[-1] == 64 and q.stride(-1) == 1
          and k.stride(-1) == 1 and v.stride(-1) == 1)
    if not ok:
        raise NotImplementedError(f"HIP attention supports head_dim 64 with contiguous head_dim; got {q.shape}")
    qb, kb, vb = (t if t.dtype == torch.bfloat16 else t.to(torch.bfloat16) for t in (q, k, v))
    out = _Attention.apply(qb, kb, vb, float(scale), bool(causal), int(q_offset))
    return out if v.dtype == torch.bfloat16 else out.to(v.dtype)


def adam(p, g, m, v, step, lr, b1, b2, eps, wd, inplace):
    assert p.dtype == torch.float32 and m.dtype == torch.float32 and v.dtype == torch.float32
    g = g.contiguous()
    if g.dtype not in (torch.float32, torch.bfloat16):
        g = g.float()
    pc, mc, vc = p.contiguous(), m.contiguous(), v.contiguous()
    if inplace and pc.data_ptr() == p.data_ptr():
        po, mo, vo = p, m, v
    else:
        po, mo, vo = torch.empty_like(pc), torch.empty_like(mc), torch.empty_like(vc)
    step_i = step if step.dtype == torch.int32 else step.to(torch.int32)
    rc = lib().ljs_adam_f32(_p(pc), _p(g), int(g.dtype == torch.bfloat16), _p(mc), _p(vc), _p(po), _p(mo), _p(vo),
                            _p(step_i), p.numel(), lr, b1, b2, eps, wd, _stream(p))
    _ck(rc, "ljs_adam_f32")
    return po.view(p.shape), mo.view(m.shape), vo.view(v.shape)


class SlabGrad:
    __slots__ = ("slabs", "S", "offset", "ld", "slab_stride", "shape")

    def __init__(self, slabs, S, offset, ld, slab_stride, shape):
        self.slabs, self.S, self.offset, self.ld, self.slab_stride = slabs, S, offset, ld, slab_stride
        self.shape = tuple(shape)


class ConstGrad:
    __slots__ = ("value", "shape")

    def __init__(self, value, shape):
        self.value, self.shape = float(value), tuple(shape)


_DEFER_INC = os.environ.get("LJS_ADAM_DEFER_INC", "1") == "1"
_PENDING_INC: Dict[int, list] = {}


def _flush_step_incs() -> None:
    while _PENDING_INC:
        _, (st, n) = _PENDING_INC.popitem()
        if n:
            _ck(lib().ljs_step_add(_p(st), n, _stream(st)), "ljs_step_add")


def flush_step_inc(step: torch.Tensor) -> None:
    ent = _PENDING_INC.get(step.data_ptr())
    if ent is not None and ent[1]:
        _ck(lib().ljs_step_add(_p(ent[0]), ent[1], _stream(ent[0])), "ljs_step_add")
        ent[1] = 0


def _defer_step_inc(step: torch.Tensor):
    if not _DEFER_INC:
        return None
    from ..spmd import graphs as _graphs
    g = _graphs.current()
    if g is None or isinstance(g, _graphs.MultiDeviceGraph):
        return None
    if _flush_step_incs not in _graphs.BEFORE_CUT:
        _graphs.BEFORE_CUT.append(_flush_step_incs)
    ent = _PENDING_INC.setdefault(step.data_ptr(), [step, 0])
    pend = ent[1]
    ent[1] += 1
    return pend




_ADAM_ROWS = [0]


def set_adam_rows(rows: int) -> None:
    lib().ljs_adam_set_rows(int(rows))
    _ADAM_ROWS[0] = int(rows)


def adam_rows() -> int:
    return _ADAM_ROWS[0]


def _grad_source(g, shape):
    import numpy as np
    shape = tuple(shape)
    R, C = (shape[0], shape[1]) if len(shape) == 2 else (1, int(math.prod(shape)))
    if isinstance(g, SlabGrad):
        assert g.shape == shape and g.slabs.dtype in (torch.float32, torch.bfloat16) \
            and g.slabs.is_contiguous()
        es = g.slabs.element_size()
        gsrc = (g.slabs.data_ptr() + es * g.offset, int(es == 2), g.S, g.ld, g.slab_stride)
    elif isinstance(g, ConstGrad):
        assert g.shape == shape
        bits = int(np.asarray(g.value, dtype=np.float32).view(np.int32))
        gsrc = (0, 0, -1, bits, 0)
    else:
        if g.dtype not in (torch.float32, torch.bfloat16) or not g.is_contiguous():
            g = g.float().contiguous() if g.dtype not in (torch.float32, torch.bfloat16) else g.contiguous()
        gsrc = (g.data_ptr(), int(g.dtype == torch.bfloat16), 0, C, 0)
    return R, C, gsrc, g


def take_step_offset(step: torch.Tensor, increment_step: bool):
    if increment_step:
        assert step.dtype == torch.int32 and step.is_contiguous()
    pend = _defer_step_inc(step) if increment_step else None
    return int(increment_step) + (pend or 0), pend


def _sumsq_ws(dev: torch.device) -> torch.Tensor:
    return _workspace(dev, "grad_sumsq", 4 * lib().ljs_grad_sumsq_ws_words())


def grad_sumsq(sources, device: torch.device) -> torch.Tensor:
    import numpy as np
    ws = _sumsq_ws(device)
    rows = []
    for shape, g in sources:
        R, C, gsrc, g = _grad_source(g, shape)
        rows.append(([0, gsrc[0], 0, 0, 0, 0, R, C, gsrc[1], gsrc[2], 0, 0, 0, 0, gsrc[3], gsrc[4]], g))
    n_launch = (len(rows) + 31) // 32
    if n_launch > lib().ljs_grad_sumsq_slots():
        raise ValueError(f"grad_sumsq: {len(rows)} tensors need {n_launch} launches; the workspace holds "
                         f"{lib().ljs_grad_sumsq_slots()} slots")
    stream = torch.cuda.current_stream(device).cuda_stream
    for k in range(n_launch):
        chunk = rows[32 * k:32 * k + 32]
        tab = np.asarray([r[0] for r in chunk], dtype=np.int64).reshape(-1)
        arr = (ctypes.c_long * tab.size)(*tab.tolist())
        _ck(lib().ljs_grad_sumsq(arr, len(chunk), _p(ws), k, stream), "ljs_grad_sumsq")
    w0 = lib().ljs_grad_sumsq_slot_word()
    return ws[w0:w0 + 2 * n_launch].view(torch.float64)


def step_hyper(step: torch.Tensor, step_offset: int, schedule=None, lr: float = 0.0, max_norm=None,
               slots: Optional[torch.Tensor] = None, gathered: Optional[torch.Tensor] = None) -> torch.Tensor:
    rec = torch.empty(4, dtype=torch.float32, device=step.device)
    kind, ps = (schedule.kind, schedule.params) if schedule is not None else (0, (float(lr), 0.0, 0.0, 0.0, 0.0))
    for t in (slots, gathered):
        assert t is None or (t.dtype == torch.float64 and t.is_contiguous() and t.device == step.device)
    rc = lib().ljs_step_hyper(_p(slots), 0 if slots is None else slots.numel(), _p(gathered),
                              0 if gathered is None else gathered.numel(), None, _p(step), int(step_offset),
                              int(max_norm is not None), float(max_norm or 0.0), int(kind), *[float(x) for x in ps],
                              _p(rec), _stream(step))
    _ck(rc, "ljs_step_hyper")
    return rec


def sumsq_partial(slots: torch.Tensor) -> torch.Tensor:
    out = torch.empty(1, dtype=torch.float64, device=slots.device)
    rc = lib().ljs_step_hyper(_p(slots), slots.numel(), None, 0, _p(out), None, 0, 0, 0.0, 0, 0.0, 0.0, 0.0, 0.0, 0.0,
                              None, _stream(slots))
    _ck(rc, "ljs_step_hyper")
    return out


def adam_multi(entries, step: torch.Tensor, lr, b1, b2, eps, wd, increment_step: bool = False,
               hyper: Optional[torch.Tensor] = None, taken=None) -> None:
    from . import shadow
    import numpy as np
    rows = []
    for p, g, m, v in entries:
        assert p.is_contiguous() and m.is_contiguous() and v.is_contiguous() and p.dtype == torch.float32
        R, C, gsrc, g = _grad_source(g, p.shape)
        bufs = shadow.kinds_of(p) if p.dim() == 2 else {}
        st, sn = bufs.get("T"), bufs.get("N")
        ptr = lambda k: bufs[k].data_ptr() if k in bufs else 0
        rows.append(([p.data_ptr(), gsrc[0], m.data_ptr(), v.data_ptr(),
                      st.data_ptr() if st is not None else 0, sn.data_ptr() if sn is not None else 0,
                      R, C, gsrc[1], gsrc[2],
                      ptr("QN"), ptr("QNs"), ptr("QT"), ptr("QTs"), gsrc[3], gsrc[4]], g))
    if increment_step:
        assert step.dtype == torch.int32 and step.is_contiguous()
    step_i = step if step.dtype == torch.int32 else step.to(torch.int32)
    offset, pend = taken if taken is not None else take_step_offset(step_i, increment_step)
    cast = None
    if rows and step_i.is_cuda:
        from . import linear as _lin
# ... 104 lines not shown
```

learning_jax_sharding_amd/ops/linear.py:

```python
from __future__ import annotations

import contextlib
import os
import threading
from typing import List, Optional, Sequence, Tuple

import numpy as np
import torch

from . import hip
from . import shadow

__all__ = ["linear"]

import weakref

_RELU_OUT = {}
_PREMASKED = {}


def _register(table, t: torch.Tensor, *extra) -> None:
    key = t.data_ptr()
    ref = weakref.ref(t, lambda _r, k=key, tb=table: tb.pop(k, None) if tb.get(k, (None,))[0] is _r else None)
    table[key] = (ref, t._version) + extra
# ... 39 lines not shown

@contextlib.contextmanager
def attention_next(heads: int, dim_head: int, scale: float):
    prev = _ATTN_NEXT[0]
    _ATTN_NEXT[0] = (int(heads), int(dim_head), float(scale)) if _QKV_ATTN else None
    try:
        yield
    finally:
        _ATTN_NEXT[0] = prev


def _fuse_attention_ok(x, xb, wt, nw, N, K, b, relu, res, od, out_dtype, wmajor, order, swap) -> Optional[tuple]:
    fz = _ATTN_NEXT[0]
    if fz is None or nw != 3 or b is not None or relu or res is not None or swap or wmajor:
        return None
    heads, dh, _ = fz
    if not (od == torch.bfloat16 and out_dtype == torch.bfloat16 and x.is_cuda and x.dim() == 3
            and order == (0, 1, 2) and x.shape[1] == 256 and dh == 64 and N == heads * 64 and K % 128 == 0
            and xb.dtype == torch.bfloat16 and xb.stride(1) == 1 and xb.stride(0) % 8 == 0
            and xb.data_ptr() % 16 == 0 and wt.is_contiguous() and wt.data_ptr() % 16 == 0):
        return None
    if 2 * (x.shape[0] * heads) < _cu_count(x.device):
        return None
    return fz


_CUS: dict = {}


def _cu_count(dev: torch.device) -> int:
    n = _CUS.get(dev.index)
    if n is None:
        n = _CUS[dev.index] = torch.cuda.get_device_properties(dev).multi_processor_count
    return n


_FUSED_SUM = os.environ.get("LJS_FUSED_SUM", "1") == "1"


_DEFER = None
_DEFER_ON = os.environ.get("LJS_DEFER_WGRAD", "1") == "1"


def _key(t: torch.Tensor):
    fn = t.grad_fn
    if fn is not None and type(fn).__name__ in _SLAB_CONSUMERS:
        return ("node", id(fn), t.output_nr)
    return (t.data_ptr(), tuple(t.shape))


_SLAB_CONSUMERS = ("_GatherBf16Backward",)


def defer_safe_leaves(outs, leaves: bool = True) -> set:
    counts, prod, seen = {}, {}, set()
    stack = [fn for fn in (t.grad_fn if isinstance(t, torch.Tensor) else t.node for t in outs) if fn is not None]
    while stack:
        fn = stack.pop()
        if id(fn) in seen:
            continue
        seen.add(id(fn))
        for nxt, idx in fn.next_functions:
            if nxt is None:
                continue
            var = getattr(nxt, "variable", None)
            k = None
            if var is not None:
                k = _key(var) if leaves else None
            elif type(nxt).__name__ in _SLAB_CONSUMERS:
                k = ("node", id(nxt), idx)
            if k is not None:
                counts[k] = counts.get(k, 0) + 1
                prod[k] = fn
            if var is None and id(nxt) not in seen:
                stack.append(nxt)
    return {k for k, c in counts.items() if c == 1 and type(prod[k]).__name__ in _DEFER_NODES}


_PROJ_ON = os.environ.get("LJS_ATTN_BWD_PROJ", "1") != "0"
_PROJ_SAFE: Optional[set] = None
_VIEW_NODES = ("ViewBackward0", "UnsafeViewBackward0", "ReshapeAliasBackward0", "AliasBackward0")


def proj_safe_nodes(outs) -> set:
    counts, seen, lins, keep = {}, set(), [], []
    roots = [(t.grad_fn, t.output_nr) if isinstance(t, torch.Tensor) else (t.node, t.output_nr) for t in outs]
    stack = []
    for fn, nr in roots:
        if fn is not None:
            counts[(id(fn), nr)] = counts.get((id(fn), nr), 0) + 1
            stack.append(fn)
    while stack:
        fn = stack.pop()
        keep.append(fn)
        if id(fn) in seen:
            continue
        seen.add(id(fn))
        if type(fn).__name__ == "_LinearBackward":
            lins.append(fn)
        for nxt, idx in fn.next_functions:
            if nxt is None:
                continue
            keep.append(nxt)
            counts[(id(nxt), idx)] = counts.get((id(nxt), idx), 0) + 1
            if id(nxt) not in seen:
                stack.append(nxt)
    safe = set()
    for fn in lins:
        nxt, idx = fn.next_functions[0]
        while nxt is not None and counts.get((id(nxt), idx), 0) == 1:
            name = type(nxt).__name__
            if name == "_AttentionBackward":
                safe.add(id(fn))
                break
            if name not in _VIEW_NODES or len(nxt.next_functions) != 1:
                break
            nxt, idx = nxt.next_functions[0]
    return safe


_DEFER_NODES = ("_LinearBackward", "_FFBlockBackward", "_FFBlockFp8Backward")


def defer_slabs(w: torch.Tensor, out: torch.Tensor, ld: int, offset: int = 0):
    d = _DEFER
    if d is None or not _defer_ok(w) or tuple(out.shape) != tuple(w.shape) or out.dtype != torch.float32:
        return None
    pend = d["pending"]

    def defer(slabs, S, mat):
        pend[out.data_ptr()] = (hip.SlabGrad(slabs, S, offset, ld, slabs[0].numel(), tuple(out.shape)), mat)
    return defer


class defer_wgrads:

    def __init__(self, outs, enabled: bool, proxies: bool = False):
        self.state = None
        if (enabled or proxies) and _DEFER_ON:
            safe = defer_safe_leaves(outs, leaves=enabled)
            if safe:
                self.state = {"safe": safe, "pending": {}}
        self.proj = (proj_safe_nodes(outs) or None) if _DEFER_ON and _PROJ_ON else None

    def __enter__(self):
        global _DEFER, _PROJ_SAFE
        self.prev, _DEFER = _DEFER, self.state
        self.prev_proj, _PROJ_SAFE = _PROJ_SAFE, self.proj
        return self

    def __exit__(self, *exc):
        global _DEFER, _PROJ_SAFE
        flush_held_dw()
        hip.materialise_out_proj()
        _DEFER = self.prev
        _PROJ_SAFE = self.prev_proj
        return False

    def take(self, g: torch.Tensor):
        if self.state is None or g is None:
            return None
        ent = self.state["pending"].pop(g.data_ptr(), None)
        if ent is None:
            return None
        if tuple(ent[0].shape) != tuple(g.shape) or g.dtype != torch.float32 or not g.is_contiguous():
            ent[1]()
            return None
        return ent

    def flush(self):
        if self.state is not None:
            for _, mat in list(self.state["pending"].values()):
                mat()
            self.state["pending"].clear()


def _defer_ok(*ts) -> bool:
    d = _DEFER
    return d is not None and all(t is not None and t.dtype == torch.float32 and _key(t) in d["safe"] for t in ts)


_SLAB_DT = torch.float32


_DW_GROUP = os.environ.get("LJS_DW_GROUP", "1") == "1"
_HELD: dict = {}
_HELD_LOCK = threading.RLock()


class _DwJob:
    __slots__ = ("K", "N", "T", "tiles", "run")

    def __init__(self, K: int, N: int, T: int, tiles: int, run):
        self.K, self.N, self.T, self.tiles, self.run = K, N, T, tiles, run

    def run_alone(self):
        tile, S, _ = hip.pick_dw_slabs(self.K, self.N, self.T)
        self.run(tile, S)


def _group_ok(ref: torch.Tensor) -> bool:
    return _DW_GROUP and _DEFER is not None and ref.is_cuda and not _DW_SPLIT


def deferred_pending():
    if _DEFER is None:
        return None
    flush_held_dw()
    return _DEFER["pending"]


def flush_held_dw():
    if not _HELD:
        return
    with _HELD_LOCK:
        while _HELD:
            _, (job, st) = _HELD.popitem()
            if st is None:
                job.run_alone()
                continue
            with torch.cuda.stream(st):
                job.run_alone()


def _hold_dw(job: _DwJob, ref: torch.Tensor) -> None:
    stream = torch.cuda.current_stream(ref.device) if ref.is_cuda else None
    with _HELD_LOCK:
        held = _HELD.pop(ref.device.index, None)
        if held is None:
            _HELD[ref.device.index] = (job, stream)
            return
        prev, pst = held
        if pst != stream:
            with torch.cuda.stream(pst):
                prev.run_alone()
            _HELD[ref.device.index] = (job, stream)
            return
        pick = hip.pick_dw_pair(prev.K, prev.N, job.K, job.N, job.T) if prev.T == job.T else None
        if pick is None:
            prev.run_alone()
            job.run_alone()
            return
        tile, s0, s1 = pick
        hip.gemm_group_begin()
        try:
            prev.run(tile, s0)
            job.run(tile, s1)
        finally:
            hip.gemm_group_end(ref)


def _dw_slabs_wmajor(xb: torch.Tensor, dys, T: int, K: int, N: int, ws, pend):
    nw = len(ws)
    tile, S, slab_mode = hip.pick_dw_slabs(K, nw * N, T)
    if not slab_mode or (_DW_SPLIT and T % (64 * _DW_SPLIT) == 0):
        return None
    out = torch.empty((nw, K, N), dtype=torch.float32, device=xb.device)
    deferred = [pend is not None and _defer_ok(w) for w in ws]

    def run(tile, S):
        slabs = torch.empty((S, nw, K, N), dtype=_SLAB_DT, device=xb.device)
        hip.gemm(xb, dys[0], slabs, K, N, T, K, N, N, False, False, batch=nw, sA=0, sC=K * N, splitk=S,
                 tile=tile, slabs=True, b_list=dys)
        done = []

        def materialize():
            if not done:
                done.append(True)
                flush_held_dw()
                hip.slab_reduce(slabs.view(S, nw * K, N), out.view(nw * K, N), N, 0)
        for i in range(nw):
            if deferred[i]:
                pend[out[i].data_ptr()] = (hip.SlabGrad(slabs, S, i * K * N, N, nw * K * N, (K, N)), materialize)
            else:
                materialize()
    if all(deferred) and _group_ok(xb):
        _hold_dw(_DwJob(K, nw * N, T, nw * -(-K // 128) * -(-N // 128), run), xb)
    else:
        run(tile, S)
    return [out[i] for i in range(nw)]


def _dw_slabs(xb: torch.Tensor, dy: torch.Tensor, ld: int, T: int, K: int, Nt: int, out: torch.Tensor, cb: int,
              out_bs: int, twin: Optional[torch.Tensor] = None, tail=None, defer=None) -> None:
    tile, S, slab_mode = hip.pick_dw_slabs(K, Nt, T)
    if _DW_SPLIT and T % (64 * _DW_SPLIT) == 0:
        S, slab_mode = _DW_SPLIT, False

    def run(tile, S):
        slabs = torch.empty((S, K, Nt), dtype=_SLAB_DT if slab_mode else torch.float32, device=xb.device)
        if slab_mode:
            hip.gemm(xb, dy, slabs, K, Nt, T, K, ld, Nt, False, False, sC=K * Nt, splitk=S, tile=tile, slabs=True)
        else:
            kc = T // S
            hip.gemm(xb, dy, slabs, K, Nt, kc, K, ld, Nt, False, False, batch=S, sA=kc * K, sB=kc * ld,
                     sC=K * Nt, tile=tile)
        done = []

        def materialize():
            if done:
                return
            done.append(True)
            flush_held_dw()
            if tail is not None:
                hip.slab_reduce(slabs, out, cb, out_bs, out_bf16=twin, tail=tail[0], tail_bf16=tail[1],
                                tail_val=tail[2])
            else:
                hip.slab_reduce(slabs, out, cb, out_bs, out_bf16=twin)
        if defer is not None:
            defer(slabs, S, materialize)
        else:
            materialize()
    if slab_mode and defer is not None and _group_ok(xb):
        _hold_dw(_DwJob(K, Nt, T, -(-K // 128) * -(-Nt // 128), run), xb)
    else:
        run(tile, S)


def _row_view(dy: torch.Tensor, M: int, N: int) -> Tuple[torch.Tensor, int]:
    d2 = dy.reshape(M, N)
    if d2.is_cuda and d2.numel() > 0 and d2.stride(0) == 0 and d2.stride(1) == 0:
        g1 = d2.as_strided((1,), (1,))
        cval = hip.seed_constant(g1)
        row = hip.const_row_bf16(cval, N, d2.device) if cval is not None else None
        if row is None:
            row, _ = hip.bcast_scalar(g1, N, M, False)
        return row.unsqueeze(0).expand(M, N), 0
    if d2.stride(0) == 0:
        row = d2[0].contiguous()
        row = _bf16(row)
        return row.unsqueeze(0).expand(M, N), 0
    if d2.stride(1) != 1 or d2.stride(0) < N:
        d2 = d2.contiguous()
    if d2.dtype != torch.bfloat16:
        d2 = _bf16(d2.contiguous())
    return d2, d2.stride(0)


_TOKEN_OUTER: List[Optional[int]] = [None]


class token_outer:

    def __init__(self, dim: Optional[int]):
        self.dim = dim

    def __enter__(self):
        self.prev, _TOKEN_OUTER[0] = _TOKEN_OUTER[0], self.dim
        return self

    def __exit__(self, *exc):
        _TOKEN_OUTER[0] = self.prev
        return False


def _inv_perm(order):
    inv = [0] * len(order)
    for i, d in enumerate(order):
        inv[d] = i
    return tuple(inv)


def _row_order(x: torch.Tensor):
    nd = x.dim()
    ident = tuple(range(nd))
    o = hip.storage_order(x) if x.is_cuda else None
    if o is not None and o[-1] == nd - 1 and o != ident:
        return tuple(o), False
    hint = _TOKEN_OUTER[0]
    if (hint == 1 and nd == 3 and x.is_cuda and x.is_contiguous() and x.shape[0] > 1 and x.shape[1] > 1
            and x.shape[2] % 8 == 0 and x.dtype in (torch.float32, torch.bfloat16) and x.data_ptr() % 16 == 0):
        return (1, 0, 2), True
    return ident, False


def _bf16(t: torch.Tensor) -> torch.Tensor:
    if t.dtype == torch.bfloat16:
        return t
    if t.is_contiguous():
        pre = _take_precast(t)
        if pre is not None:
            return pre
        return hip._cast_raw(t, torch.bfloat16)
    return t.to(torch.bfloat16)


_PRECAST_MODE = os.environ.get("LJS_PRECAST", "join")
_NEXT_INPUTS: List[torch.Tensor] = []
_PLAIN_CAST = set()
PRECAST_STATS = {"taken": 0}
_PRECAST = {}
_OPT_PRECAST = os.environ.get("LJS_OPT_PRECAST", "1")


def _pc_key(t: torch.Tensor):
    return (t.data_ptr(), t.numel(), t._version, t.device.index)


def prefetch_next_input(*xs) -> None:
# ... 126 lines not shown
                           sC=M * N if wmajor else N, bias=bias, sBias=0, relu=relu, psum=partials, res=r2,
                           res_ld=r_ld)
        cols = [out[i] if wmajor else out[:, i * N:(i + 1) * N] for i in range(nw)]
        ys = [c.view(pshape + (N,)).permute(inv) for c in cols]
        if res is not None and r2 is None:
            ys = [ys[0] + res.to(ys[0].dtype)]
            partials = None
        if partials is not None and cnt > 0 and od == out_dtype:
            hip._register_psum(ys[0], partials, cnt)
        if od != out_dtype:
            ys = [y.to(out_dtype) for y in ys]
        if relu and od == torch.bfloat16:
            for y in ys:
                _register(_RELU_OUT, y)
        ctx.premask = bool(xb.dtype == torch.bfloat16 and K % 8 == 0 and _is_relu_out(xb) and _relu_node(x))
        ctx.has_res = res is not None
        ctx.save_for_backward(xb, b, *ws, *(ys if relu else []))
        ctx.meta = (lead, K, M, N, nw, relu, x.dtype, b is not None)
        ctx.order, ctx.pshape = order, pshape
        return tuple(ys)

    @staticmethod
    def backward(ctx, *dys):
        lead, K, M, N, nw, relu, xdtype, has_b = ctx.meta
        order = getattr(ctx, "order", None)
        pshape = ctx.pshape if order is not None else tuple(lead)
        if order is None:
            order = tuple(range(len(lead) + 1))
        dres = dys[0] if (ctx.has_res and ctx.needs_input_grad[2]) else None
        dys = tuple(None if d is None else d.permute(order) for d in dys)
        saved = ctx.saved_tensors
        xb, b = saved[0], saved[1]
        ctx.bias_leaf = b
        ws = saved[2:2 + nw]
        ys = tuple(y.permute(order) for y in saved[2 + nw:]) if relu else None
        dev = xb.device
        mats: List[Optional[Tuple[torch.Tensor, int]]] = []
        db_bcast: List[Optional[torch.Tensor]] = [None] * nw
        want_db = has_b and ctx.needs_input_grad[1]
        from ..parallel import data as _dp
        wire = _dp.active_wire_dtype() == torch.bfloat16
        joint = joint_bf16 = tail = None
        if (nw == 1 and want_db and ctx.needs_input_grad[5] and dys[0] is not None and M % 64 == 0 and not relu
                and b.dtype == torch.float32 and ws[0].dtype == torch.float32 and dys[0].is_cuda
                and dys[0].numel() > 0 and all(st == 0 for st in dys[0].stride())):
            joint = torch.empty((K * N + N,), dtype=torch.float32, device=dev)
            joint_bf16 = torch.empty((K * N + N,), dtype=torch.bfloat16, device=dev) if wire else None
        for i, dy in enumerate(dys):
            if dy is None:
                mats.append(None)
                continue
            if relu and _premasked_by(dy, ys[i]):
                mats.append(_row_view(dy, M, N))
                continue
            if relu:
                d2, y2 = dy.reshape(M, N), ys[i].reshape(M, N)
                if (d2.is_cuda and d2.dtype == torch.bfloat16 and y2.dtype == torch.bfloat16 and N % 8 == 0
                        and d2.stride(1) == 1 and y2.stride(1) == 1 and d2.stride(0) % 8 == 0
                        and y2.stride(0) % 8 == 0 and d2.data_ptr() % 16 == 0 and y2.data_ptr() % 16 == 0):
                    if want_db:
                        masked, db_bcast[i] = hip.relu_bwd_colsum(d2, y2, M, N)
                    else:
                        masked = hip.relu_bwd(d2, y2, M, N)
                    mats.append((masked, N))
                    continue
                dy = (dy * (ys[i] > 0)).reshape(M, N)
            elif dy.is_cuda and dy.numel() > 0 and all(st == 0 for st in dy.stride()):
                g1 = dy.as_strided((1,), (1,))
                cval = hip.seed_constant(g1) if joint is not None else None
                row = hip.const_row_bf16(cval, N, dev) if cval is not None else None
                if row is not None:
                    db_bcast[i] = joint[K * N:]
                    tail = (joint[K * N:], joint_bf16[K * N:] if joint_bf16 is not None else None,
                            float(np.float32(cval) * np.float32(M)))
                    mats.append((row.unsqueeze(0).expand(M, N), 0))
                    continue
                row, db_bcast[i] = hip.bcast_scalar(
                    dy.as_strided((1,), (1,)), N, M, want_db,
                    db_out=joint[K * N:] if joint is not None else None,
                    db_bf16=joint_bf16[K * N:] if joint_bf16 is not None else None)
                mats.append((row.unsqueeze(0).expand(M, N), 0))
                continue
            mats.append(_row_view(dy, M, N))
        dx = db = None
        dws = [None] * nw
        live = [i for i in range(nw) if mats[i] is not None]
        if ctx.needs_input_grad[0] and live:
            out_dt = torch.bfloat16 if (xdtype == torch.bfloat16 and len(live) == 1) else torch.float32
            dx = torch.empty((M, K), dtype=out_dt, device=dev)
            premask = ctx.premask and out_dt == torch.bfloat16
            hand_over = (_PROJ_SAFE is not None and id(ctx) in _PROJ_SAFE and len(live) == 1 and nw == 1
                         and out_dt == torch.bfloat16 and not relu and not premask and dx.is_cuda
                         and tuple(order) == tuple(range(len(order))))
            for j, i in enumerate(live):
                t, ld = mats[i]
                wn = shadow.get(ws[i], "N")
                if hand_over:
                    hip.defer_out_proj(t, ld, wn, dx, lambda t=t, ld=ld, wn=wn, dx=dx: hip.gemm(
                        t, wn, dx, M, K, N, ld, N, K, True, True))
                    continue
                hip.gemm(t, wn, dx, M, K, N, ld, N, K, True, True, accumulate=j > 0,
                         res=xb if premask else None, res_ld=K, res_mode="mask")
            dx = dx.to(xdtype).view(pshape + (K,)).permute(_inv_perm(order))
            if premask:
                _register(_PREMASKED, dx, xb.data_ptr())
        want = [i for i in live if ctx.needs_input_grad[5 + i]]
        _wgrads(ctx, xb, ws, mats, want, dws, joint, joint_bf16, K, M, N, nw, wire, dev, tail)
        if want_db and live:
            tot = None
            for i in live:
                if db_bcast[i] is not None:
                    tot = db_bcast[i] if tot is None else tot + db_bcast[i]
                    continue
                t, ld = mats[i]
                pre = hip.colsum_for(t, N) if ld > 0 else None
                if pre is not None:
                    tot = pre if tot is None else tot + pre
                    continue
                tot = hip.colsum_ld(t, M, N, ld, tot)
            db = tot.to(b.dtype)
        if joint is not None:
            if dws[0] is None or db is None or db.data_ptr() != joint[K * N:].data_ptr():
                joint_bf16 = None
            if joint_bf16 is not None:
                _dp.register_wire_twin(joint, joint_bf16)
        return (dx, db, dres, None, None, *dws)


_PENDING_WAITS: List = []


def defer_wait(handle) -> None:
    _PENDING_WAITS.append(handle)


def take_pending_waits(dev) -> None:
    while _PENDING_WAITS:
        _PENDING_WAITS.pop().wait()


def twin_free(joint_bf16, wire) -> bool:
    return joint_bf16 is None and not wire


def _wgrads(ctx, xb, ws, mats, want, dws, joint, joint_bf16, K, M, N, nw, wire, dev, tail=None):
    from ..parallel import data as _dp
    if not want:
        return
    t0, ld0 = mats[want[0]]
    batched = (len(want) == nw and nw > 1 and ld0 > 0 and all(
        mats[i][1] == ld0 and mats[i][0].data_ptr() == t0.data_ptr() + i * N * 2 for i in want))
    dma = M % 64 == 0
    if dma:
        pend = _DEFER["pending"] if _DEFER is not None and twin_free(joint_bf16, wire) else None
        if joint is not None:
            t, ld = mats[0]
            dW = joint[:K * N].view(K, N)
            defer = None
            if pend is not None and _defer_ok(ws[0], *([ctx.bias_leaf] if tail is not None else [])):
                def defer(slabs, S, mat, dW=dW):
                    pend[dW.data_ptr()] = (hip.SlabGrad(slabs, S, 0, N, K * N, (K, N)), mat)
                    if tail is not None:
                        pend[tail[0].data_ptr()] = (hip.ConstGrad(tail[2], (N,)), mat)
            _dw_slabs(xb, t, ld, M, K, N, dW, N, 0,
                      joint_bf16[:K * N].view(K, N) if joint_bf16 is not None else None, tail, defer)
            dws[0] = dW
        elif batched:
            dW = torch.empty((nw, K, N), dtype=torch.float32, device=dev)
            twin = torch.empty((nw, K, N), dtype=torch.bfloat16, device=dev) if wire else None
            defer = None
            if pend is not None and twin is None and _defer_ok(*[ws[i] for i in want]):
                def defer(slabs, S, mat, dW=dW):
                    for i in want:
                        pend[dW[i].data_ptr()] = (hip.SlabGrad(slabs, S, i * N, nw * N, K * nw * N, (K, N)), mat)
            _dw_slabs(xb, t0, ld0, M, K, nw * N, dW, N, K * N, twin, defer=defer)
            if twin is not None:
                _dp.register_wire_twin(dW, twin)
            for i in want:
                dws[i] = dW[i] if ws[i].dtype == torch.float32 else dW[i].to(ws[i].dtype)
        elif (_WMAJOR_BATCH and len(want) == nw and 1 < nw <= 4 and not wire and all(
                mats[i][1] == N and mats[i][0].stride(-1) == 1 and mats[i][0].data_ptr() % 16 == 0 for i in want)
                and (wm := _dw_slabs_wmajor(xb, [mats[i][0] for i in want], M, K, N, [ws[i] for i in want],
                                            pend)) is not None):
            for j, i in enumerate(want):
                dws[i] = wm[j] if ws[i].dtype == torch.float32 else wm[j].to(ws[i].dtype)
        else:
            for i in want:
                t, ld = mats[i]
                dW = torch.empty((K, N), dtype=torch.float32, device=dev)
                twin = torch.empty((K, N), dtype=torch.bfloat16, device=dev) if wire else None
                defer = None
                if pend is not None and twin is None and _defer_ok(ws[i]):
                    def defer(slabs, S, mat, dW=dW):
                        pend[dW.data_ptr()] = (hip.SlabGrad(slabs, S, 0, N, K * N, (K, N)), mat)
                _dw_slabs(xb, t, ld, M, K, N, dW, N, 0, twin, defer=defer)
                if twin is not None:
                    _dp.register_wire_twin(dW, twin)
                dws[i] = dW if ws[i].dtype == torch.float32 else dW.to(ws[i].dtype)
    else:
        tile = 128 if (K >= 256 and N >= 256) else 64
        if batched:
            dW = torch.empty((nw, K, N), dtype=torch.float32, device=dev)
            sk = _splitk(K, N, M, nw, tile)
            hip.gemm(xb, t0, dW, K, N, M, K, ld0, N, False, False, batch=nw, sA=0, sB=N, sC=K * N,
                     splitk=sk, tile=tile, zero_c=True)
            for i in want:
                dws[i] = dW[i] if ws[i].dtype == torch.float32 else dW[i].to(ws[i].dtype)
        else:
            for i in want:
                t, ld = mats[i]
                dW = torch.empty((K, N), dtype=torch.float32, device=dev)
                sk = _splitk(K, N, M, 1, tile)
                hip.gemm(xb, t, dW, K, N, M, K, ld, N, False, False, splitk=sk, tile=tile, zero_c=True)
                dws[i] = dW if ws[i].dtype == torch.float32 else dW.to(ws[i].dtype)


_WMAJOR_BATCH = os.environ.get("LJS_WMAJOR_DW_BATCH", "1") == "1"


def supported(x: torch.Tensor, ws: Sequence[torch.Tensor], b) -> bool:
    K = x.shape[-1]
    N = ws[0].shape[1]
    M = x.numel() // max(1, K)
    return (K % 8 == 0 and N % 8 == 0 and M % 8 == 0 and all(w.shape == ws[0].shape and w.dim() == 2 for w in ws)
            and all(w.dtype == torch.float32 and w.stride(1) == 1 for w in ws)
            and (b is None or len(ws) == 1))


def linear(x: torch.Tensor, ws: List[torch.Tensor], b: Optional[torch.Tensor], relu: bool,
           out_dtype: torch.dtype, residual: Optional[torch.Tensor] = None) -> List[torch.Tensor]:
    if residual is not None and (relu or len(ws) != 1):
        ys = list(_Linear.apply(x, b, None, relu, out_dtype, *ws))
        return [ys[0] + residual.to(ys[0].dtype)] + ys[1:]
    return list(_Linear.apply(x, b, residual, relu, out_dtype, *ws))


class _FFBlock(torch.autograd.Function):

    @staticmethod
    def forward(ctx, x, w_in, w_out, res):
        M = x.shape[-1]
        F = w_in.shape[1]
        nd = x.dim()
        o = hip.storage_order(x) if x.is_cuda else None
        order = tuple(o) if o is not None and o[-1] == nd - 1 else tuple(range(nd))
        xs = x.permute(order)
        pshape = tuple(xs.shape[:-1])
        x2 = _bf16(xs.reshape(-1, M).contiguous())
        T = x2.shape[0]
        a = torch.empty((T, F), dtype=torch.bfloat16, device=x.device)
        hip.gemm(x2, shadow.get(w_in, "T"), a, T, F, M, M, M, F, True, True, relu=True)
        y = torch.empty((T, M), dtype=torch.bfloat16, device=x.device)
        hip.gemm(a, shadow.get(w_out, "T"), y, T, M, F, F, F, M, True, True, res=x2 if res else None, res_ld=M)
        ctx.save_for_backward(x2, a, w_in, w_out)
        ctx.meta = (order, pshape, M, F, T, bool(res), x.dtype)
        return y.view(pshape + (M,)).permute(_inv_perm(order))

    @staticmethod
    def backward(ctx, dy):
        from ..parallel import data as _dp
        x2, a, w_in, w_out = ctx.saved_tensors
        order, pshape, M, F, T, res, xdt = ctx.meta
        dev = x2.device
        t, ld = _row_view(dy.permute(order), T, M)
        wire = _dp.active_wire_dtype() == torch.bfloat16
        dA = torch.empty((T, F), dtype=torch.bfloat16, device=dev)
        hip.gemm(t, shadow.get(w_out, "N"), dA, T, F, M, ld, M, F, True, True, res=a, res_ld=F, res_mode="mask")
        out = {}

        def run_dx():
            if ctx.needs_input_grad[0]:
                dx = torch.empty((T, M), dtype=torch.bfloat16, device=dev)
                hip.gemm(dA, shadow.get(w_in, "N"), dx, T, M, F, F, F, M, True, True, res=t if res else None,
                         res_ld=ld)
                out["dx"] = dx.to(xdt).view(pshape + (M,)).permute(_inv_perm(order))

        def wgrad(xb, g, g_ld, K, N, w):
            o = torch.empty((K, N), dtype=torch.float32, device=dev)
# ... 39 lines not shown
```

Measured before the change: 748.1 TFLOPS, whole job (matmul FLOPs of fwd+bwd summed over the n_gpus GPUs; the per-GPU rate the metric names is tflops_per_gpu = value / n_gpus).

## Replace broadcast-dy output-projection weight gradient with a fused rank-1 form

```diff
diff --git a/learning_jax_sharding_amd/csrc/kernels/adam_common.h b/learning_jax_sharding_amd/csrc/kernels/adam_common.h
--- a/learning_jax_sharding_amd/csrc/kernels/adam_common.h
+++ b/learning_jax_sharding_amd/csrc/kernels/adam_common.h
@@ -24,13 +24,16 @@
   t.gS = r[9]; t.g_ld = r[14]; t.g_ss = r[15];
   if (t.gS == 0) t.g_ld = t.C;
   if (t.gS > 0 && (t.g_ld < t.C || t.g_ss < 1)) return false;
+  if (t.gS < -2 || (t.gS == -2 && (!t.g || t.g % 4 || !t.g_ss || t.g_ss % 2 || t.g_ld < 1 || t.g_bf16 < t.R)))
+    return false;
   t.tiles_c = (t.C + 63) / 64;
   return true;
 }
 inline bool adam_grad_vec_ok(const AdamTensor& t) {
   auto al = [](long ptr, long a) { return ptr % a == 0; };
   return t.C % 4 == 0 &&
-         (t.gS < 0 || (al(t.g, t.g_bf16 ? 8 : 16) && t.g_ld % 4 == 0 && (t.gS == 0 || t.g_ss % 4 == 0)));
+         (t.gS == -1 || (t.gS == -2 && al(t.g_ss, 8)) ||
+          (t.gS >= 0 && al(t.g, t.g_bf16 ? 8 : 16) && t.g_ld % 4 == 0 && (t.gS == 0 || t.g_ss % 4 == 0)));
 }
 
 template <typename ST>
@@ -58,6 +61,49 @@
   return acc;
 }
 
+template <int NR>
+__device__ __forceinline__ void rank1_tile_u(const AdamTensor& T, long row0, float* stage, float* ush) {
+  static_assert(NR == 16 || NR == 32 || NR == 64, "tile height");
+  constexpr int NL = NR * 64 / 256;
+  const float* __restrict__ parts = reinterpret_cast<const float*>(T.g);
+  const long P = T.g_ld, ps = T.g_bf16;
+  const int tid = threadIdx.x;
+  float u = 0.f;
+  for (long p0 = 0; p0 < P; p0 += 64) {
+    const int r = tid % NR, pq = tid / NR;
+    const bool rok = row0 + r < T.R;
+    const float* src = parts + (p0 + pq) * ps + row0 + r;
+    float v[NL];
+#pragma unroll
+    for (int k = 0; k < NL; ++k)
+      v[k] = (rok && p0 + pq + (256 / NR) * k < P) ? src[(long)(256 / NR) * k * ps] : 0.f;
+#pragma unroll
+    for (int k = 0; k < NL; ++k) stage[r * 65 + pq + (256 / NR) * k] = v[k];
+    __syncthreads();
+    if (tid < NR) {
+      const int n = (int)(P - p0 < 64 ? P - p0 : 64);
+      int p = 0;
+      if (p0 == 0) {
+        u = stage[tid * 65];
+        p = 1;
+      }
+#pragma unroll 8
+      for (; p < n; ++p) u += stage[tid * 65 + p];
+    }
+    __syncthreads();
+  }
+  if (tid < NR) ush[tid] = u;
+  __syncthreads();
+}
+__device__ __forceinline__ float rank1_mul(float u, float c) { return __fmul_rn(u, c); }
+__device__ __forceinline__ float rank1_g1(const AdamTensor& T, float u, long col) {
+  return rank1_mul(u, bf2f(reinterpret_cast<const bf16_t*>(T.g_ss)[col]));
+}
+__device__ __forceinline__ f32x4 rank1_g4(const AdamTensor& T, float u, long col) {
+  const f32x4 c = unpack_bf16x4(*reinterpret_cast<const u32x2*>(reinterpret_cast<const bf16_t*>(T.g_ss) + col));
+  return f32x4{rank1_mul(u, c[0]), rank1_mul(u, c[1]), rank1_mul(u, c[2]), rank1_mul(u, c[3])};
+}
+
 struct StepHyper {
   float grad_scale, lr, norm, pad;
 };
diff --git a/learning_jax_sharding_amd/csrc/kernels/attention.hip b/learning_jax_sharding_amd/csrc/kernels/attention.hip
--- a/learning_jax_sharding_amd/csrc/kernels/attention.hip
+++ b/learning_jax_sharding_amd/csrc/kernels/attention.hip
@@ -1550,7 +1550,7 @@
 #endif
 }
 
-__device__ __forceinline__ void fused_delta(const bf16_t* Ot, const bf16_t* dOt, float* ndl, int tid) {
+__device__ __forceinline__ u32x4 fused_delta(const bf16_t* Ot, const bf16_t* dOt, float* ndl, int tid) {
   const int row = tid >> 3, c16 = tid & 7;
   const u32x4 o = *reinterpret_cast<const u32x4*>(Ot + img16(row, c16));
   const u32x4 d = *reinterpret_cast<const u32x4*>(dOt + img16(row, c16));
@@ -1559,6 +1559,38 @@
   s += __shfl_xor(s, 2, 64);
   s += __shfl_xor(s, 4, 64);
   if (c16 == 0) ndl[row] = -s;
+  return o;
+}
+
+__device__ __forceinline__ void osum_add(const u32x4& o, float (&os)[8]) {
+#pragma unroll
+  for (int i = 0; i < 4; ++i) {
+    os[2 * i] += __uint_as_float(o[i] << 16);
+    os[2 * i + 1] += __uint_as_float(o[i] & 0xffff0000u);
+  }
+}
+__device__ __forceinline__ void osum_stage(float* img, float (&os)[8], int tid) {
+  const int lane = tid & 63, wave = tid >> 6;
+#pragma unroll
+  for (int e = 0; e < 8; ++e) {
+    float s = os[e];
+    s += __shfl_xor(s, 8, 64);
+    s += __shfl_xor(s, 16, 64);
+    s += __shfl_xor(s, 32, 64);
+    os[e] = s;
+  }
+  if (lane < 8) {
+    *reinterpret_cast<f32x4*>(img + wave * D + 8 * lane) = f32x4{os[0], os[1], os[2], os[3]};
+    *reinterpret_cast<f32x4*>(img + wave * D + 8 * lane + 4) = f32x4{os[4], os[5], os[6], os[7]};
+  }
+}
+__device__ __forceinline__ void osum_flush(const float* img, float* __restrict__ dst, int tid) {
+  if (tid < 64) {
+    float s = img[tid];
+#pragma unroll
+    for (int w = 1; w < FT / 64; ++w) s += img[w * D + tid];
+    dst[tid] = s;
+  }
 }
 
 template <bool GUARD>
@@ -1772,6 +1804,7 @@
   long dy_ld;
   int M;
   unsigned long long* steps;
+  float* osum;
 };
 constexpr int PJ_TS = 32;
 constexpr int PJ_BK = 32;
@@ -1787,7 +1820,7 @@
 constexpr int PJB_ROW = 2048;
 static_assert((PJB_NST & (PJB_NST - 1)) == 0 && PJB_NST * PJB_STAGE <= PJ_Q - PJ_DST, "the stages fit the two images");
 static_assert((PJ_LDS + PJB_ROW) * 2 <= 160 * 1024, "LDS");
-template <bool BCAST>
+template <bool BCAST, bool OSUM>
 __global__ __launch_bounds__(FT) void attn_bwd_proj_kernel(AttnArgs a, BwdProjArgs pj) {
   __shared__ __attribute__((aligned(16))) bf16_t smem[PJ_LDS + (BCAST ? PJB_ROW : 0)];
   bf16_t* const Ks = smem + PJ_KS;
@@ -1825,7 +1858,12 @@
     dma_lds_x4_at(ro, (int)(((long)r * a.o_ss + dchunk) * 2), sb + 2 * (PJ_OS + wave * 512));
     if (wave == 0) dma_lds_x1_at(rl, (q0 + lane) * 4, sb + 2 * PJ_ROWC + 4 * (buf * 2 * BLK));
   };
-  auto finish = [&](int buf, int blk) { fused_delta(Os, dOi + blk * BLK * D, rowc + (buf * 2 + 1) * BLK, tid); };
+  [[maybe_unused]] float os[8] = {};
+  auto finish = [&](int buf, int blk) {
+    const u32x4 o = fused_delta(Os, dOi + blk * BLK * D, rowc + (buf * 2 + 1) * BLK, tid);
+    if constexpr (OSUM) osum_add(o, os);
+    else (void)o;
+  };
 
   {
     const int nk = pj.M / PJ_BK;
@@ -2023,11 +2061,15 @@
     asm volatile("s_waitcnt vmcnt(0)" ::: "memory");
     __syncthreads();
     if (more) finish(cur ^ 1, it + 1);
+    if constexpr (OSUM)
+      if (!more) osum_stage(reinterpret_cast<float*>(Os), os, tid);
     f32x4 dq[2] = {};
     fused_dq<false>(Ks, dSt, dq, off_q, off_k, FK / 32);
     fused_dq_stage(dOt, dq, a.scale, qt, dt0, lane);
     __syncthreads();
     fused_dq_flush<false>(a, dOt, b, h, q0, tid);
+    if constexpr (OSUM)
+      if (!more) osum_flush(reinterpret_cast<const float*>(Os), pj.osum + ((long)b * a.H + h) * D, tid);
     bstamp(2 + it);
   }
   fused_dkv_out(a, Ks, Vs, dk, dv, b, h, key0, FK, lane);
@@ -2376,13 +2418,15 @@
                               const void* w, int M, const void* lse, void* dq, void* dk, void* dv, int B, int Sq,
                               int Sk, int H, const long* qs, const long* ks, const long* vs, const long* os,
                               const long* dqs, const long* dks, const long* dvs, float scale, int causal,
-                              hipStream_t stream, AttnPlan* plan = nullptr) {
+                              hipStream_t stream, AttnPlan* plan = nullptr, void* osum = nullptr) {
   if (!none_null({qs, ks, vs, os, dqs, dks, dvs})) return (int)hipErrorInvalidValue;
+  if (osum && (dy_ld != 0 || ((uintptr_t)osum & 15))) return (int)hipErrorInvalidValue;
   AttnArgs a = attn_outs(attn_args(q, k, v, o, lse, qs, ks, vs, os, Sq, Sk, H, scale, causal, 0), dk, dks, dv, dvs,
                          dq, dqs);
   BwdProjArgs pj;
   pj.dy = (const bf16_t*)dy; pj.w = (const bf16_t*)w; pj.dy_ld = dy_ld; pj.M = M;
   pj.steps = g_attn_trace_steps;
+  pj.osum = (float*)osum;
   const AttnPlan p = attn_bwd_proj_plan(a, B, pj);
   if (plan) *plan = p;
   if (plan || p.err != hipSuccess) return (int)p.err;
@@ -2391,8 +2435,11 @@
   ljs_launch_rec(kAttnInst[kBwdProj].name, dim3(p.l[0].gx), p.l[0].block);
   const bool bcast = dy_ld == 0 && M <= PJB_ROW && bwd_proj_bcast_on();
   g_bwd_proj_last_path = bcast;
-  if (bcast) hipLaunchKernelGGL(attn_bwd_proj_kernel<true>, dim3(p.l[0].gx), dim3(p.l[0].block), 0, stream, a, pj);
-  else hipLaunchKernelGGL(attn_bwd_proj_kernel<false>, dim3(p.l[0].gx), dim3(p.l[0].block), 0, stream, a, pj);
+  const dim3 grid(p.l[0].gx), block(p.l[0].block);
+  if (bcast && osum) hipLaunchKernelGGL((attn_bwd_proj_kernel<true, true>), grid, block, 0, stream, a, pj);
+  else if (bcast) hipLaunchKernelGGL((attn_bwd_proj_kernel<true, false>), grid, block, 0, stream, a, pj);
+  else if (osum) hipLaunchKernelGGL((attn_bwd_proj_kernel<false, true>), grid, block, 0, stream, a, pj);
+  else hipLaunchKernelGGL((attn_bwd_proj_kernel<false, false>), grid, block, 0, stream, a, pj);
   return (int)hipGetLastError();
 }
 LJS_API int ljs_attn_bwd_proj_last_path() { return g_bwd_proj_last_path; }
@@ -2403,6 +2450,14 @@
                               hipStream_t stream) {
   return attn_bwd_proj_impl(q, k, v, o, dy, dy_ld, w, M, lse, dq, dk, dv, B, Sq, Sk, H, qs, ks, vs, os, dqs, dks, dvs,
                             scale, causal, stream);
+}
+LJS_API int ljs_attn_bwd_proj_osum(const void* q, const void* k, const void* v, const void* o, const void* dy,
+                                   long dy_ld, const void* w, int M, const void* lse, void* dq, void* dk, void* dv,
+                                   int B, int Sq, int Sk, int H, const long* qs, const long* ks, const long* vs,
+                                   const long* os, const long* dqs, const long* dks, const long* dvs, float scale,
+                                   int causal, void* osum, hipStream_t stream) {
+  return attn_bwd_proj_impl(q, k, v, o, dy, dy_ld, w, M, lse, dq, dk, dv, B, Sq, Sk, H, qs, ks, vs, os, dqs, dks, dvs,
+                            scale, causal, stream, nullptr, osum);
 }
 
 LJS_API int ljs_attn_plan(int kind, int B, int Sq, int Sk, int H, int causal, int acc_mode, void* const* addr,
diff --git a/learning_jax_sharding_amd/csrc/kernels/clip.hip b/learning_jax_sharding_amd/csrc/kernels/clip.hip
--- a/learning_jax_sharding_amd/csrc/kernels/clip.hip
+++ b/learning_jax_sharding_amd/csrc/kernels/clip.hip
@@ -37,7 +37,9 @@
     const bool bf = T.g_bf16 != 0;
     const int local = id - batch.tile_start[ti];
     const int tr_i = local / (int)T.tiles_c, tc_i = local % (int)T.tiles_c;
-    if (gS >= 0 && T.vec && (long)(tc_i + 1) * 64 <= C) {
+    __shared__ float stage[kSumsqRows * 65], ush[kSumsqRows];
+    if (gS == -2) rank1_tile_u<kSumsqRows>(T, (long)tr_i * kSumsqRows, stage, ush);
+    if ((gS >= 0 || gS == -2) && T.vec && (long)(tc_i + 1) * 64 <= C) {
       const long cbase = (long)tc_i * 64 + c4;
       f32x4 g[2];
       bool ok[2];
@@ -46,7 +48,9 @@
         const long row = (long)tr_i * kSumsqRows + r0 + 16 * q;
         ok[q] = row < R;
         const long gi = (ok[q] ? row : 0) * g_ld + cbase;
-        if (gS > 0) {
+        if (gS == -2) {
+          g[q] = rank1_g4(T, ush[r0 + 16 * q], cbase);
+        } else if (gS > 0) {
           g[q] = bf ? slab_sum4(reinterpret_cast<const bf16_t*>(T.g), gS, g_ss, gi)
                     : slab_sum4(reinterpret_cast<const float*>(T.g), gS, g_ss, gi);
         } else {
@@ -67,6 +71,7 @@
         const long gi = row * g_ld + col;
         const float g = gS > 0   ? (bf ? slab_sum1(reinterpret_cast<const bf16_t*>(T.g), gS, g_ss, gi)
                                        : slab_sum1(reinterpret_cast<const float*>(T.g), gS, g_ss, gi))
+                        : gS == -2 ? rank1_g1(T, ush[w + 4 * rr], col)
                         : gS < 0 ? __int_as_float((int)g_ld)
                         : bf     ? bf2f(reinterpret_cast<const bf16_t*>(T.g)[gi])
                                  : reinterpret_cast<const float*>(T.g)[gi];
diff --git a/learning_jax_sharding_amd/csrc/kernels/elementwise.hip b/learning_jax_sharding_amd/csrc/kernels/elementwise.hip
--- a/learning_jax_sharding_amd/csrc/kernels/elementwise.hip
+++ b/learning_jax_sharding_amd/csrc/kernels/elementwise.hip
@@ -473,6 +473,7 @@
                                                          std::conditional_t<kDyn, const StepHyper*, float> lr_arg,
                                                          float b1, float b2, float eps, float wd, CastJob cast) {
   __shared__ float tr[kAdamRows][65];
+  __shared__ float ush[kAdamRows];
   float lr;
   [[maybe_unused]] float gscale = 1.f;
   if constexpr (kDyn) {
@@ -529,6 +530,7 @@
       vv[q] = *(const __attribute__((address_space(1))) f32x4*)(Vv + i);
       pv[q] = *(const __attribute__((address_space(1))) f32x4*)(P + i);
     }
+    if (T.gS == -2) rank1_tile_u<TR>(T, (long)tr_i * TR, &tr[0][0], ush);
     if (T.gS > 0) {
       auto slab_sum = [&](auto tag) {
         using ST = decltype(tag);
@@ -600,6 +602,8 @@
     for (int q = 0; q < NQ; ++q) {
       const long gi = gix[q];
       if (T.gS > 0) {
+      } else if (T.gS == -2) {
+        gv[q] = rank1_g4(T, ush[r0 + RPP * q], cbase);
       } else if (T.gS < 0) {
         const float c = __int_as_float((int)T.g_ld);
         gv[q] = f32x4{c, c, c, c};
@@ -694,6 +698,7 @@
     }
     return;
   }
+  if (T.gS == -2) rank1_tile_u<kAdamRows>(T, (long)tr_i * kAdamRows, &tr[0][0], ush);
 #pragma unroll 4
   for (int rr = 0; rr < kAdamRows / (kThreads / 64); ++rr) {
     const int rl = ty + (kThreads / 64) * rr, row = tr_i * kAdamRows + rl;
@@ -703,6 +708,7 @@
       const long gi = (long)row * T.g_ld + col;
       float g = T.gS > 0   ? (T.g_bf16 ? slab_sum1(reinterpret_cast<const bf16_t*>(T.g), T.gS, T.g_ss, gi)
                                         : slab_sum1(reinterpret_cast<const float*>(T.g), T.gS, T.g_ss, gi))
+                : T.gS == -2 ? rank1_g1(T, ush[rl], col)
                 : T.gS < 0 ? __int_as_float((int)T.g_ld)
                 : T.g_bf16 ? bf2f(reinterpret_cast<const bf16_t*>(T.g)[gi])
                            : reinterpret_cast<const float*>(T.g)[gi];
@@ -1103,6 +1109,59 @@
   return (int)hipGetLastError();
 }
 
+__global__ __launch_bounds__(256) void rank1_expand_kernel(AdamTensor T, float* __restrict__ out,
+                                                           bf16_t* __restrict__ out_bf16, float* __restrict__ tail,
+                                                           bf16_t* __restrict__ tail_bf16, int tail_n, float tail_val) {
+  if (blockIdx.x == 0) {
+    for (int i = threadIdx.x; i < tail_n; i += blockDim.x) {
+      tail[i] = tail_val;
+      if (tail_bf16) tail_bf16[i] = f2bf(tail_val);
+    }
+  }
+  const int tr_i = blockIdx.x / (int)T.tiles_c, tc_i = blockIdx.x % (int)T.tiles_c;
+  __shared__ float stage[32 * 65], ush[32];
+  rank1_tile_u<32>(T, (long)tr_i * 32, stage, ush);
+  if (T.vec && (long)(tc_i + 1) * 64 <= T.C) {
+    const long col = (long)tc_i * 64 + (threadIdx.x & 15) * 4;
+#pragma unroll
+    for (int q = 0; q < 2; ++q) {
+      const int rl = (threadIdx.x >> 4) + 16 * q;
+      const long row = (long)tr_i * 32 + rl;
+      if (row >= T.R) continue;
+      const f32x4 g = rank1_g4(T, ush[rl], col);
+      *reinterpret_cast<f32x4*>(out + row * T.C + col) = g;
+      if (out_bf16)
+        *reinterpret_cast<u32x2*>(out_bf16 + row * T.C + col) = u32x2{pack_bf16x2(g[0], g[1]), pack_bf16x2(g[2], g[3])};
+    }
+    return;
+  }
+  const long col = (long)tc_i * 64 + (threadIdx.x & 63);
+  for (int rr = 0; rr < 8; ++rr) {
+    const int rl = (threadIdx.x >> 6) + 4 * rr;
+    const long row = (long)tr_i * 32 + rl;
+    if (row < T.R && col < T.C) {
+      const float g = rank1_g1(T, ush[rl], col);
+      out[row * T.C + col] = g;
+      if (out_bf16) out_bf16[row * T.C + col] = f2bf(g);
+    }
+  }
+}
+
+LJS_API int ljs_rank1_expand(const long* row, void* out, void* out_bf16, void* tail, void* tail_bf16, int tail_n,
+                             float tail_val, hipStream_t s) {
+  AdamTensor t = AdamTensor{};
+  if (!row || !out || tail_n < 0 || (tail_n > 0 && !tail) || !adam_grad_from_row(row, t) || t.gS != -2 || t.R < 1 ||
+      t.C < 1)
+    return (int)hipErrorInvalidValue;
+  t.vec = adam_grad_vec_ok(t) && ((uintptr_t)out & 15) == 0 && ((uintptr_t)out_bf16 & 7) == 0;
+  const long tiles = ((t.R + 31) / 32) * t.tiles_c;
+  if (tiles > 0x7fffffffL) return (int)hipErrorInvalidValue;
+  ljs_launch_rec("rank1_expand", dim3((unsigned)tiles), 256);
+  hipLaunchKernelGGL(rank1_expand_kernel, dim3((unsigned)tiles), dim3(256), 0, s, t, (float*)out, (bf16_t*)out_bf16,
+                     (float*)tail, (bf16_t*)tail_bf16, tail_n, tail_val);
+  return (int)hipGetLastError();
+}
+
 LJS_API int ljs_bcast_scalar(const void* g, int g_bf16, int C, float R, void* row, void* db, void* db_bf16,
                              hipStream_t s) {
   hipLaunchKernelGGL(bcast_scalar_kernel, dim3((C + 255) / 256), dim3(256), 0, s, g, g_bf16, C, R, (bf16_t*)row,
diff --git a/learning_jax_sharding_amd/ops/hip.py b/learning_jax_sharding_amd/ops/hip.py
--- a/learning_jax_sharding_amd/ops/hip.py
+++ b/learning_jax_sharding_amd/ops/hip.py
@@ -50,6 +50,9 @@
     "ljs_attn_bwd_proj": [c_void_p, c_void_p, c_void_p, c_void_p, c_void_p, c_long, c_void_p, c_int, c_void_p,
                           c_void_p, c_void_p, c_void_p, c_int, c_int, c_int, c_int, _LP, _LP, _LP, _LP, _LP, _LP, _LP,
                           c_float, c_int, c_void_p],
+    "ljs_attn_bwd_proj_osum": [c_void_p, c_void_p, c_void_p, c_void_p, c_void_p, c_long, c_void_p, c_int, c_void_p,
+                               c_void_p, c_void_p, c_void_p, c_int, c_int, c_int, c_int, _LP, _LP, _LP, _LP, _LP, _LP,
+                               _LP, c_float, c_int, c_void_p, c_void_p],
     "ljs_attn_bwd_proj_enabled": [c_int, c_int],
     "ljs_attn_bwd_proj_last_path": [],
     "ljs_cast_f32_bf16": [c_void_p, c_void_p, c_long, c_void_p],
@@ -69,6 +72,7 @@
                     c_int, c_void_p],
     "ljs_slab_reduce": [c_void_p, c_int, c_long, c_int, c_int, c_void_p, c_int, c_long, c_int, c_void_p, c_void_p,
                         c_void_p, c_int, c_float, c_int, c_void_p],
+    "ljs_rank1_expand": [_LP, c_void_p, c_void_p, c_void_p, c_void_p, c_int, c_float, c_void_p],
     "ljs_softmax_rows_f32": [c_void_p, c_void_p, c_long, c_int, c_void_p],
     "ljs_adam_f32": [c_void_p, c_void_p, c_int, c_void_p, c_void_p, c_void_p, c_void_p, c_void_p, c_void_p, c_long,
                      c_float, c_float, c_float, c_float, c_float, c_void_p],
@@ -1812,7 +1816,7 @@
 FUSED_ATTN_STATS = {"taken": 0}
 
 
-_PROJ_PENDING: Dict[int, tuple] = {}
+_PROJ_PENDING: Dict[int, list] = {}
 ATTN_BWD_PROJ_STATS = {"taken": 0, "materialised": 0}
 
 
@@ -1833,16 +1837,21 @@
 
 
 def attn_bwd_proj_block(q, k, v, o, dy: torch.Tensor, dy_ld: int, w: torch.Tensor, lse, scale: float,
-                        causal: bool = False, outs=None):
+                        causal: bool = False, outs=None, osum: Optional[torch.Tensor] = None):
     B, Sq, H, D = q.shape
     if outs is None:
         outs = tuple(torch.empty((B, Sq, H, D), dtype=torch.bfloat16, device=q.device) for _ in range(3))
     dq, dk, dv = outs
-    rc = lib().ljs_attn_bwd_proj(_p(q), _p(k), _p(v), _p(o), _p(dy), int(dy_ld), _p(w), int(w.shape[1]), _p(lse),
-                                 _p(dq), _p(dk), _p(dv), B, Sq, k.shape[1], H, _longs(_strides3(q)),
-                                 _longs(_strides3(k)), _longs(_strides3(v)), _longs(_strides3(o)),
-                                 _longs(_strides3(dq)), _longs(_strides3(dk)), _longs(_strides3(dv)), float(scale),
-                                 int(causal), _stream(q))
+    args = (_p(q), _p(k), _p(v), _p(o), _p(dy), int(dy_ld), _p(w), int(w.shape[1]), _p(lse),
+            _p(dq), _p(dk), _p(dv), B, Sq, k.shape[1], H, _longs(_strides3(q)),
+            _longs(_strides3(k)), _longs(_strides3(v)), _longs(_strides3(o)),
+            _longs(_strides3(dq)), _longs(_strides3(dk)), _longs(_strides3(dv)), float(scale), int(causal))
+    if osum is None:
+        rc = lib().ljs_attn_bwd_proj(*args, _stream(q))
+    else:
+        assert osum.dtype == torch.float32 and tuple(osum.shape) == (B, H * D) and osum.is_contiguous() \
+            and osum.device == q.device
+        rc = lib().ljs_attn_bwd_proj_osum(*args, _p(osum), _stream(q))
     _ck(rc, "ljs_attn_bwd_proj")
     return dq, dk, dv
 
@@ -1856,13 +1865,45 @@
     if materialise_out_proj not in _graphs.BEFORE_CUT:
         _graphs.BEFORE_CUT.append(materialise_out_proj)
         _graphs.AFTER_CAPTURE.append(materialise_out_proj)
-    _PROJ_PENDING[dx.data_ptr()] = (dy, ld, wn, dx, launch)
+    _PROJ_PENDING[dx.data_ptr()] = [dy, ld, wn, dx, launch, None]
+
+
+class Rank1Request:
+    __slots__ = ("parts", "x", "fallback", "state")
+
+    def __init__(self, parts: torch.Tensor, x: torch.Tensor, fallback):
+        self.parts, self.x, self.fallback, self.state = parts, x, fallback, "open"
+
+    def take(self, o: torch.Tensor) -> Optional[torch.Tensor]:
+        B, Sq, H, D = o.shape
+        if (o.data_ptr() == self.x.data_ptr() and o.is_contiguous() and self.x.is_contiguous()
+                and o.dtype == self.x.dtype and tuple(self.x.shape) == (B * Sq, H * D)
+                and tuple(self.parts.shape) == (B, H * D)):
+            self.state = "taken"
+            RANK1_STATS["used"] += 1
+            return self.parts
+        self.fall()
+        return None
+
+    def fall(self) -> None:
+        if self.state == "open":
+            self.state = "fallen"
+            self.fallback()
+
+
+RANK1_STATS = {"used": 0}
+
+
+def attach_rank1(dx: torch.Tensor, req: Rank1Request) -> None:
+    _PROJ_PENDING[dx.data_ptr()][5] = req
 
 
 def materialise_out_proj() -> None:
     while _PROJ_PENDING:
         _, ent = _PROJ_PENDING.popitem()
         ent[4]()
+        if ent[5] is not None:
+            ent[5].fall()
         ATTN_BWD_PROJ_STATS["materialised"] += 1
 
 
@@ -1870,13 +1911,18 @@
     ent = _PROJ_PENDING.pop(do.data_ptr(), None)
     if ent is None:
         return None
-    dy, ld, wn, dx, launch = ent
+    dy, ld, wn, dx, launch, rank1 = ent
     B, Sq, H, D = q.shape
     if (do.dtype == torch.bfloat16 and tuple(do.shape) == (B, Sq, H, D) and do.is_contiguous()
             and dx.numel() == do.numel() and attn_bwd_proj_ok(q, k, v, o, dy, ld, wn, causal, outs)):
         ATTN_BWD_PROJ_STATS["taken"] += 1
-        return dy, ld, wn
+        osum = None
+        if rank1 is not None:
+            osum = rank1.take(o) if ld == 0 else rank1.fall()
+        return dy, ld, wn, osum
     launch()
+    if rank1 is not None:
+        rank1.fall()
     ATTN_BWD_PROJ_STATS["materialised"] += 1
     return None
 
@@ -1939,7 +1985,8 @@
             dv = _bs_like((B, Sk, H, D), v)
         proj = _take_out_proj(do, q, k, v, o, (dq, dk, dv), causal) if _PROJ_PENDING else None
         if proj is not None:
-            attn_bwd_proj_block(q, k, v, o, proj[0], proj[1], proj[2], lse, scale, causal, outs=(dq, dk, dv))
+            attn_bwd_proj_block(q, k, v, o, proj[0], proj[1], proj[2], lse, scale, causal, outs=(dq, dk, dv),
+                                osum=proj[3])
         else:
             _attn_bwd_call(q, k, v, o, do, lse, dq, dk, dv, scale, causal, q_offset)
         return dq.to(q.dtype), dk.to(k.dtype), dv.to(v.dtype), None, None, None
@@ -2017,6 +2064,36 @@
         self.value, self.shape = float(value), tuple(shape)
 
 
+class Rank1Grad:
+    __slots__ = ("parts", "P", "row", "shape")
+
+    def __init__(self, parts, P, row, shape):
+        self.parts, self.P, self.row, self.shape = parts, int(P), row, tuple(shape)
+        R, C = self.shape
+        assert parts.dtype == torch.float32 and parts.is_contiguous() and tuple(parts.shape) == (self.P, R)
+        assert row.dtype == torch.bfloat16 and row.is_contiguous() and tuple(row.shape) == (C,) \
+            and row.device == parts.device
+
+
+def rank1_expand(g: Rank1Grad, out: torch.Tensor, out_bf16: Optional[torch.Tensor] = None,
+                 tail: Optional[torch.Tensor] = None, tail_bf16: Optional[torch.Tensor] = None,
+                 tail_val: float = 0.0) -> None:
+    R, C, gsrc, _ = _grad_source(g, g.shape)
+    assert out.dtype == torch.float32 and out.is_contiguous() and tuple(out.shape) == (R, C)
+    assert out_bf16 is None or (out_bf16.dtype == torch.bfloat16 and out_bf16.is_contiguous()
+                                and out_bf16.numel() == out.numel())
+    tn = 0
+    if tail is not None:
+        assert tail.dtype == torch.float32 and tail.is_contiguous() and tail.device == out.device
+        assert tail_bf16 is None or (tail_bf16.dtype == torch.bfloat16 and tail_bf16.numel() == tail.numel()
+                                     and tail_bf16.is_contiguous())
+        tn = tail.numel()
+    row = _longs([0, gsrc[0], 0, 0, 0, 0, R, C, gsrc[1], gsrc[2], 0, 0, 0, 0, gsrc[3], gsrc[4]])
+    rc = lib().ljs_rank1_expand(row, _p(out), _p(out_bf16), _p(tail), _p(tail_bf16 if tn else None), tn,
+                                float(tail_val), _stream(out))
+    _ck(rc, "rank1_expand")
+
+
 _DEFER_INC = os.environ.get("LJS_ADAM_DEFER_INC", "1") == "1"
 _PENDING_INC: Dict[int, list] = {}
 
@@ -2077,6 +2154,9 @@
         assert g.shape == shape
         bits = int(np.asarray(g.value, dtype=np.float32).view(np.int32))
         gsrc = (0, 0, -1, bits, 0)
+    elif isinstance(g, Rank1Grad):
+        assert g.shape == shape and len(shape) == 2
+        gsrc = (g.parts.data_ptr(), R, -2, g.P, g.row.data_ptr())
     else:
         if g.dtype not in (torch.float32, torch.bfloat16) or not g.is_contiguous():
             g = g.float().contiguous() if g.dtype not in (torch.float32, torch.bfloat16) else g.contiguous()
diff --git a/learning_jax_sharding_amd/ops/linear.py b/learning_jax_sharding_amd/ops/linear.py
--- a/learning_jax_sharding_amd/ops/linear.py
+++ b/learning_jax_sharding_amd/ops/linear.py
@@ -145,6 +145,13 @@
 _VIEW_NODES = ("ViewBackward0", "UnsafeViewBackward0", "ReshapeAliasBackward0", "AliasBackward0")
 
 
+class _ProjSafe(set):
+
+    def __init__(self, *a):
+        super().__init__(*a)
+        self.attn = {}
+
+
 def proj_safe_nodes(outs) -> set:
     counts, seen, lins, keep = {}, set(), [], []
     roots = [(t.grad_fn, t.output_nr) if isinstance(t, torch.Tensor) else (t.node, t.output_nr) for t in outs]
@@ -168,13 +175,14 @@
             counts[(id(nxt), idx)] = counts.get((id(nxt), idx), 0) + 1
             if id(nxt) not in seen:
                 stack.append(nxt)
-    safe = set()
+    safe = _ProjSafe()
     for fn in lins:
         nxt, idx = fn.next_functions[0]
         while nxt is not None and counts.get((id(nxt), idx), 0) == 1:
             name = type(nxt).__name__
             if name == "_AttentionBackward":
                 safe.add(id(fn))
+                safe.attn[id(fn)] = nxt
                 break
             if name not in _VIEW_NODES or len(nxt.next_functions) != 1:
                 break
@@ -279,6 +287,8 @@
     with _HELD_LOCK:
         while _HELD:
             _, (job, st) = _HELD.popitem()
+            if job.run is None:
+                continue
             if st is None:
                 job.run_alone()
                 continue
@@ -294,23 +304,45 @@
             _HELD[ref.device.index] = (job, stream)
             return
         prev, pst = held
+        ghost = prev.run is None
         if pst != stream:
-            with torch.cuda.stream(pst):
-                prev.run_alone()
+            if not ghost:
+                with torch.cuda.stream(pst):
+                    prev.run_alone()
             _HELD[ref.device.index] = (job, stream)
             return
         pick = hip.pick_dw_pair(prev.K, prev.N, job.K, job.N, job.T) if prev.T == job.T else None
         if pick is None:
-            prev.run_alone()
+            if not ghost:
+                prev.run_alone()
             job.run_alone()
             return
         tile, s0, s1 = pick
+        if ghost:
+            job.run(tile, s1)
+            return
         hip.gemm_group_begin()
         try:
             prev.run(tile, s0)
             job.run(tile, s1)
         finally:
             hip.gemm_group_end(ref)
+
+
+def _hold_ghost(ghost: _DwJob, ref: torch.Tensor) -> bool:
+    stream = torch.cuda.current_stream(ref.device) if ref.is_cuda else None
+    with _HELD_LOCK:
+        if ref.device.index in _HELD:
+            return False
+        _HELD[ref.device.index] = (ghost, stream)
+        return True
+
+
+def _drop_ghost(ghost: _DwJob, ref: torch.Tensor) -> None:
+    with _HELD_LOCK:
+        held = _HELD.get(ref.device.index)
+        if held is not None and held[0] is ghost:
+            del _HELD[ref.device.index]
 
 
 def _dw_slabs_wmajor(xb: torch.Tensor, dys, T: int, K: int, N: int, ws, pend):
@@ -345,7 +377,7 @@
 
 
 def _dw_slabs(xb: torch.Tensor, dy: torch.Tensor, ld: int, T: int, K: int, Nt: int, out: torch.Tensor, cb: int,
-              out_bs: int, twin: Optional[torch.Tensor] = None, tail=None, defer=None) -> None:
+              out_bs: int, twin: Optional[torch.Tensor] = None, tail=None, defer=None, job_only: bool = False):
     tile, S, slab_mode = hip.pick_dw_slabs(K, Nt, T)
     if _DW_SPLIT and T % (64 * _DW_SPLIT) == 0:
         S, slab_mode = _DW_SPLIT, False
@@ -374,10 +406,81 @@
             defer(slabs, S, materialize)
         else:
             materialize()
+    if job_only:
+        if defer is None:
+            return None
+        if not slab_mode:
+            return (lambda: run(tile, S)), None
+        job = _DwJob(K, Nt, T, -(-K // 128) * -(-Nt // 128), run)
+        return job.run_alone, (job if _group_ok(xb) else None)
     if slab_mode and defer is not None and _group_ok(xb):
         _hold_dw(_DwJob(K, Nt, T, -(-K // 128) * -(-Nt // 128), run), xb)
     else:
         run(tile, S)
+
+
+def _dw_rank1_on() -> bool:
+    return os.environ.get("LJS_DW_RANK1", "1") != "0"
+
+
+def dw_rank1_wanted(hand_over: bool, ld: int, deferred: bool, pairs: int, knob: Optional[bool] = None) -> bool:
+    knob = _dw_rank1_on() if knob is None else knob
+    return bool(hand_over and ld == 0 and deferred and pairs >= 192 and knob)
+
+
+def _proj_pairs(node, M: int, K: int, N: int) -> int:
+    try:
+        q, k = node.saved_tensors[:2]
+        B, Sq, H, D = q.shape
+        causal = bool(node.args[1])
+    except Exception:
+        return 0
+    if B * Sq != M or H * D != K or not hip.proj_shape_ok(B, Sq, k.shape[1], H, D, N, 0, causal):
+        return 0
+    return B * H
+
+
+def _dw_rank1(xb, t, K, N, dW, dx, pairs, tail, pend, hold) -> bool:
+    slab_mat = []
+
+    def defer(slabs, S, smat):
+        slab_mat.append(smat)
+        pend[dW.data_ptr()] = (hip.SlabGrad(slabs, S, 0, N, K * N, (K, N)), mat)
+        if tail is not None:
+            pend[tail[0].data_ptr()] = (hip.ConstGrad(tail[2], (N,)), mat)
+    held = hold(defer)
+    if held is None:
+        return False
+    alone, job = held
+    if job is not None:
+        ghost = _DwJob(job.K, job.N, job.T, job.tiles, None)
+        if not _hold_ghost(ghost, xb):
+            return False
+        run_job = alone
+
+        def alone():
+            _drop_ghost(ghost, xb)
+            run_job()
+    B = pairs // (K // 64)
+    parts = torch.empty((B, K), dtype=torch.float32, device=xb.device)
+    desc = hip.Rank1Grad(parts, B, t, (K, N))
+    req = hip.Rank1Request(parts, xb, alone)
+    done = []
+
+    def mat():
+        if req.state == "open":
+            hip.materialise_out_proj()
+        if req.state == "fallen":
+            slab_mat[0]()
+        elif not done:
+            done.append(True)
+            hip.rank1_expand(desc, dW, tail=tail[0] if tail else None, tail_bf16=tail[1] if tail else None,
+                             tail_val=tail[2] if tail else 0.0)
+    hip.attach_rank1(dx, req)
+    pend[dW.data_ptr()] = (desc, mat)
+    if tail is not None:
+        pend[tail[0].data_ptr()] = (hip.ConstGrad(tail[2], (N,)), mat)
+    return True
 
 
 def _row_view(dy: torch.Tensor, M: int, N: int) -> Tuple[torch.Tensor, int]:
@@ -670,7 +773,7 @@
                 mats.append((row.unsqueeze(0).expand(M, N), 0))
                 continue
             mats.append(_row_view(dy, M, N))
-        dx = db = None
+        dx = db = proj = None
         dws = [None] * nw
         live = [i for i in range(nw) if mats[i] is not None]
         if ctx.needs_input_grad[0] and live:
@@ -680,6 +783,8 @@
             hand_over = (_PROJ_SAFE is not None and id(ctx) in _PROJ_SAFE and len(live) == 1 and nw == 1
                          and out_dt == torch.bfloat16 and not relu and not premask and dx.is_cuda
                          and tuple(order) == tuple(range(len(order))))
+            if hand_over:
+                proj = (dx, _PROJ_SAFE.attn.get(id(ctx)))
             for j, i in enumerate(live):
                 t, ld = mats[i]
                 wn = shadow.get(ws[i], "N")
@@ -693,7 +798,7 @@
             if premask:
                 _register(_PREMASKED, dx, xb.data_ptr())
         want = [i for i in live if ctx.needs_input_grad[5 + i]]
-        _wgrads(ctx, xb, ws, mats, want, dws, joint, joint_bf16, K, M, N, nw, wire, dev, tail)
+        _wgrads(ctx, xb, ws, mats, want, dws, joint, joint_bf16, K, M, N, nw, wire, dev, tail, proj)
         if want_db and live:
             tot = None
             for i in live:
@@ -731,7 +836,7 @@
     return joint_bf16 is None and not wire
 
 
-def _wgrads(ctx, xb, ws, mats, want, dws, joint, joint_bf16, K, M, N, nw, wire, dev, tail=None):
+def _wgrads(ctx, xb, ws, mats, want, dws, joint, joint_bf16, K, M, N, nw, wire, dev, tail=None, proj=None):
     from ..parallel import data as _dp
     if not want:
         return
@@ -741,6 +846,14 @@
     dma = M % 64 == 0
     if dma:
         pend = _DEFER["pending"] if _DEFER is not None and twin_free(joint_bf16, wire) else None
+
+        def rank1(t, ld, dW, deferred, tail):
+            if proj is None or nw != 1 or not dw_rank1_wanted(True, ld, deferred, 192):
+                return False
+            pairs = _proj_pairs(proj[1], M, K, N)
+            return dw_rank1_wanted(True, ld, deferred, pairs) and _dw_rank1(
+                xb, t[0], K, N, dW, proj[0], pairs, tail, pend,
+                lambda defer: _dw_slabs(xb, t, ld, M, K, N, dW, N, 0, None, tail, defer, job_only=True))
         if joint is not None:
             t, ld = mats[0]
             dW = joint[:K * N].view(K, N)
@@ -750,8 +863,9 @@
                     pend[dW.data_ptr()] = (hip.SlabGrad(slabs, S, 0, N, K * N, (K, N)), mat)
                     if tail is not None:
                         pend[tail[0].data_ptr()] = (hip.ConstGrad(tail[2], (N,)), mat)
-            _dw_slabs(xb, t, ld, M, K, N, dW, N, 0,
-                      joint_bf16[:K * N].view(K, N) if joint_bf16 is not None else None, tail, defer)
+            if not rank1(t, ld, dW, defer is not None, tail):
+                _dw_slabs(xb, t, ld, M, K, N, dW, N, 0,
+                          joint_bf16[:K * N].view(K, N) if joint_bf16 is not None else None, tail, defer)
             dws[0] = dW
         elif batched:
             dW = torch.empty((nw, K, N), dtype=torch.float32, device=dev)
@@ -781,7 +895,8 @@
                 if pend is not None and twin is None and _defer_ok(ws[i]):
                     def defer(slabs, S, mat, dW=dW):
                         pend[dW.data_ptr()] = (hip.SlabGrad(slabs, S, 0, N, K * N, (K, N)), mat)
-                _dw_slabs(xb, t, ld, M, K, N, dW, N, 0, twin, defer=defer)
+                if not rank1(t, ld, dW, defer is not None and ws[i].dtype == torch.float32, None):
+                    _dw_slabs(xb, t, ld, M, K, N, dW, N, 0, twin, defer=defer)
                 if twin is not None:
                     _dp.register_wire_twin(dW, twin)
                 dws[i] = dW if ws[i].dtype == torch.float32 else dW.to(ws[i].dtype)
```

Result: slower. 733.1 TFLOPS, whole job (matmul FLOPs of fwd+bwd summed over the n_gpus GPUs; the per-GPU rate the metric names is tflops_per_gpu = value / n_gpus) (-2.0%).
